# LiyaoTang/contrastBoundary

Hardware: AMD Instinct MI355X
Metric: points/sec through KNN+group+KPConv+CBL block, S3DIS N=40960 K=16 (higher is better)
Workload: dtype f32

## Files before the change

contrastboundary_amd/build.py:

```python
import concurrent.futures
import os
import shutil
import subprocess
import sys

PKG = os.path.dirname(os.path.abspath(__file__))
CSRC = os.path.join(PKG, "csrc")
LIBDIR = os.path.join(PKG, "lib")
OBJDIR = os.path.join(LIBDIR, "obj")
SO = os.path.join(LIBDIR, "libcbl_amd.so")
INCLUDE = os.path.join(os.path.dirname(PKG), "include")

HIPCC = shutil.which("hipcc") or "/opt/rocm/bin/hipcc"
FLAGS = ["--offload-arch=gfx950", "-O3", "-std=c++17", "-fPIC", "-ffp-contract=off", "-munsafe-fp-atomics",
         "-fvisibility=hidden", "-Wall", "-Wno-unused-function", "-I" + INCLUDE, "-I" + CSRC]


def sources():
    return sorted(os.path.join(CSRC, f) for f in os.listdir(CSRC) if f.endswith(".hip"))


def headers():
    hs = [os.path.join(CSRC, f) for f in os.listdir(CSRC) if f.endswith(".h")]
    hs += [os.path.join(INCLUDE, f) for f in os.listdir(INCLUDE) if f.endswith(".h")]
    return hs


EXTRA_FLAGS = {"local_aggregation.hip": ["-mllvm", "-amdgpu-mfma-vgpr-form"]}

def _compile(src, obj, verbose):
    tmp = obj + ".tmp.%d" % os.getpid()
    cmd = [HIPCC] + FLAGS + EXTRA_FLAGS.get(os.path.basename(src), []) + ["-c", src, "-o", tmp]
    if verbose:
        print(" ".join(cmd), flush=True)
    r = subprocess.run(cmd, capture_output=True, text=True)
    if r.returncode != 0:
        raise RuntimeError("hipcc failed for %s:\n%s\n%s" % (src, r.stdout, r.stderr))
    if verbose and r.stderr.strip():
        print(r.stderr)
    os.replace(tmp, obj)


def is_stale():
    if not os.path.exists(SO):
        return True
    t = os.path.getmtime(SO)
    return any(os.path.getmtime(p) > t for p in sources() + headers())


def build(force=False, verbose=False):
    import fcntl
    os.makedirs(OBJDIR, exist_ok=True)
    with open(os.path.join(LIBDIR, ".build.lock"), "w") as lock:
        fcntl.flock(lock, fcntl.LOCK_EX)
        try:
            if not force and not is_stale():
                return SO
            return _build_locked(force, verbose)
        finally:
            fcntl.flock(lock, fcntl.LOCK_UN)


def _build_locked(force, verbose):
    hdr_time = max([os.path.getmtime(h) for h in headers()] + [os.path.getmtime(__file__)])
    jobs, objs = [], []
    for src in sources():
        obj = os.path.join(OBJDIR, os.path.basename(src)[:-4] + ".o")
        objs.append(obj)
        if force or not os.path.exists(obj) or os.path.getmtime(obj) < max(os.path.getmtime(src), hdr_time):
            jobs.append((src, obj))
    if jobs:
        with concurrent.futures.ThreadPoolExecutor(max_workers=min(8, len(jobs))) as ex:
            for f in [ex.submit(_compile, s, o, verbose) for s, o in jobs]:
                f.result()
    if jobs or not os.path.exists(SO):
        tmp = SO + ".tmp.%d" % os.getpid()
        cmd = [HIPCC, "--offload-arch=gfx950", "-shared", "-fPIC", "-o", tmp] + objs
        if verbose:
            print(" ".join(cmd), flush=True)
        r = subprocess.run(cmd, capture_output=True, text=True)
        if r.returncode != 0:
            raise RuntimeError("link failed:\n%s\n%s" % (r.stdout, r.stderr))
        os.replace(tmp, SO)
    else:
        os.utime(SO)
    return SO


if __name__ == "__main__":
    print(build(force="--force" in sys.argv, verbose="--verbose" in sys.argv))
```

contrastboundary_amd/csrc/local_aggregation.hip:

```cpp
#include "cbl_common.h"

namespace {

using f32x4 = __attribute__((ext_vector_type(4))) float;

template <bool VEC>
__global__ __launch_bounds__(256) void kpconv_fwd_kernel(int n, int n0, int K, int C, int KP, const float* __restrict__ q,
                                                         const float* __restrict__ s, const int* __restrict__ idx, const float* __restrict__ f,
                                                         const float* __restrict__ kpts, const float* __restrict__ kw, float extent,
                                                         int influence, int closest, const int* __restrict__ order, float* __restrict__ out)
{
    const int lane = threadIdx.x & 63;
    const int kp_id = lane & 15;
    const int kq = lane >> 4;
    const unsigned wv = __builtin_amdgcn_readfirstlane(threadIdx.x >> 6), nwg = ((unsigned)n + 3u) >> 2;
    const bool kp_ok = kp_id < KP;
    const float kx = kp_ok ? kpts[3 * kp_id] : 0.f, ky = kp_ok ? kpts[3 * kp_id + 1] : 0.f, kz = kp_ok ? kpts[3 * kp_id + 2] : 0.f;

    const float inv_extent = 1.0f / extent;
    const unsigned vend = 8 * cbl_xcd_per(nwg), vstep = gridDim.x;
    auto point_at = [&](unsigned v) -> int {
        if (v >= vend) return -1;
        const unsigned t = (order ? cbl_xcd_slot(v, nwg) : v) * 4 + wv;
        return t < (unsigned)n ? (order ? order[t] : (int)t) : -1;
    };
    struct Geo { int id; float sx, sy, sz, qx, qy, qz; };
    auto fetch_ids = [&](int pt, Geo& g) {
        g.id = (lane < K) ? idx[(size_t)pt * K + lane] : n0;
        g.qx = q[3 * pt]; g.qy = q[3 * pt + 1]; g.qz = q[3 * pt + 2];
    };
    auto fetch_xyz = [&](Geo& g) {
        const bool real = g.id >= 0 && g.id < n0;
        const float3 sp = *reinterpret_cast<const float3*>(s + 3 * (size_t)(real ? g.id : 0));
        g.sx = real ? sp.x : 1e6f; g.sy = real ? sp.y : 1e6f; g.sz = real ? sp.z : 1e6f;
    };
    int p0 = point_at(blockIdx.x), p1 = point_at(blockIdx.x + vstep);
    Geo cur = {n0, 1e6f, 1e6f, 1e6f, 0.f, 0.f, 0.f};
    if (p0 >= 0) { fetch_ids(p0, cur); fetch_xyz(cur); }
    for (unsigned v = blockIdx.x; v < vend; v += vstep) {
        const int p2 = point_at(v + 2 * vstep);
        Geo nxt = {n0, 1e6f, 1e6f, 1e6f, 0.f, 0.f, 0.f};
        if (p1 >= 0) fetch_ids(p1, nxt);
        const int p = p0;
        const Geo g = cur;
        auto advance = [&]() { if (p1 >= 0) fetch_xyz(nxt); cur = nxt; p0 = p1; p1 = p2; };
        if (p < 0) { advance(); continue; }
        const float qx = g.qx, qy = g.qy, qz = g.qz;
        for (int c0 = 0; c0 < C; c0 += 64) {
            f32x4 acc[4];
#pragma unroll
            for (int t = 0; t < 4; t++) acc[t] = f32x4{0.f, 0.f, 0.f, 0.f};
            const int cb = c0 + 4 * kp_id;
            for (int k0 = 0; k0 < K; k0 += 64) {
                int my_id; float mrx, mry, mrz;
                if (k0 == 0) { my_id = g.id; mrx = g.sx - qx; mry = g.sy - qy; mrz = g.sz - qz; }
                else {
                    const int my_nb = k0 + lane;
                    my_id = (my_nb < K) ? idx[(size_t)p * K + my_nb] : n0;
                    const bool my_real = my_id >= 0 && my_id < n0;
                    mrx = (my_real ? s[3 * my_id] : 1e6f) - qx; mry = (my_real ? s[3 * my_id + 1] : 1e6f) - qy; mrz = (my_real ? s[3 * my_id + 2] : 1e6f) - qz;
                }
                const int kend = min(64, K - k0);
                for (int kc = 0; kc < kend; kc += 16) {
                    float bv[4][4]; float a[4];
#pragma unroll
                    for (int g = 0; g < 4; g++) {
                        const int src = kc + 4 * g + kq;
                        const int id = __shfl(my_id, src & 63);
                        const bool in = (kc + 4 * g + kq) < kend;
                        const bool real = in && id >= 0 && id < n0;
#pragma unroll
                        for (int t = 0; t < 4; t++) bv[g][t] = 0.f;
                        if (real) {
                            if (VEC) {
                                if (cb < C) { const float4 v = *reinterpret_cast<const float4*>(f + (size_t)id * C + cb); bv[g][0] = v.x; bv[g][1] = v.y; bv[g][2] = v.z; bv[g][3] = v.w; }
                            } else {
#pragma unroll
                                for (int t = 0; t < 4; t++) if (cb + t < C) bv[g][t] = f[(size_t)id * C + cb + t];
                            }
                        }
                        const float rx = __shfl(mrx, src & 63), ry = __shfl(mry, src & 63), rz = __shfl(mrz, src & 63);
                        const float dx = rx - kx, dy = ry - ky, dz = rz - kz;
                        const float sq = (dx * dx + dy * dy) + dz * dz;
                        float w = influence ? fmaxf(1.0f - __builtin_amdgcn_sqrtf(sq) * inv_extent, 0.0f) : 1.0f;
                        if (closest) {
                            float bs = kp_ok ? sq : INFINITY; int bi = kp_id;
#pragma unroll
                            for (int sft = 8; sft >= 1; sft >>= 1) {
                                const float os = __shfl_xor(bs, sft, 16); const int oi = __shfl_xor(bi, sft, 16);
                                if (os < bs || (os == bs && oi < bi)) { bs = os; bi = oi; }
                            }
                            if (bi != kp_id) w = 0.f;
                        }
                        a[g] = (kp_ok && in) ? w : 0.f;
                    }
#pragma unroll
                    for (int g = 0; g < 4; g++)
#pragma unroll
                        for (int t = 0; t < 4; t++) acc[t] = __builtin_amdgcn_mfma_f32_16x16x4f32(a[g], bv[g][t], acc[t], 0, 0, 0);
                }
            }
            float res[4];
#pragma unroll
            for (int t = 0; t < 4; t++) {
                float part = 0.f;
#pragma unroll
                for (int r = 0; r < 4; r++) {
                    const int row = kq * 4 + r;
                    const float kwv = (row < KP && cb + t < C) ? kw[(size_t)row * C + cb + t] : 0.f;
                    part += kwv * acc[t][r];
                }
                part += __shfl_xor(part, 16);
                part += __shfl_xor(part, 32);
                res[t] = part;
            }
            if (lane < 16) {
                if (VEC) { if (cb < C) *reinterpret_cast<float4*>(out + (size_t)p * C + cb) = make_float4(res[0], res[1], res[2], res[3]); }
                else {
#pragma unroll
                    for (int t = 0; t < 4; t++) if (cb + t < C) out[(size_t)p * C + cb + t] = res[t];
                }
            }
        }
        advance();
    }
}

__device__ __forceinline__ float rows_sum4(float x)
{
    const unsigned u = __float_as_uint(x);
    const auto a = __builtin_amdgcn_permlane16_swap(u, u, false, false);
    const float y = __uint_as_float(a[0]) + __uint_as_float(a[1]);
    const unsigned w = __float_as_uint(y);
    const auto b = __builtin_amdgcn_permlane32_swap(w, w, false, false);
    return __uint_as_float(b[0]) + __uint_as_float(b[1]);
}

template <bool CLOSEST, bool LINEAR, bool ONE>
__global__ __launch_bounds__(256) void kpconv_fwd_c64_kernel(int n, int n0, int K, int C, int KP, const float* __restrict__ q,
                                                             const float* __restrict__ s, const int* __restrict__ idx, const float* __restrict__ f,
                                                             const float* __restrict__ kpts, const float* __restrict__ kw, float extent,
                                                             const int* __restrict__ order, float* __restrict__ out)
{
    __shared__ float4 kw_s[16 * 16];
    {
        const int row = threadIdx.x >> 4, col = threadIdx.x & 15;
        kw_s[threadIdx.x] = (row < KP && 4 * col < C) ? *reinterpret_cast<const float4*>(kw + (size_t)row * C + 4 * col) : make_float4(0.f, 0.f, 0.f, 0.f);
    }
    __syncthreads();
    const int lane = threadIdx.x & 63;
    const int kp_id = lane & 15, kq = lane >> 4;
    const unsigned wv = __builtin_amdgcn_readfirstlane(threadIdx.x >> 6), nwg = ((unsigned)n + 3u) >> 2;
    const bool kp_ok = kp_id < KP;
    const float kx = kp_ok ? kpts[3 * kp_id] : 0.f, ky = kp_ok ? kpts[3 * kp_id + 1] : 0.f, kz = kp_ok ? kpts[3 * kp_id + 2] : 0.f;
    const float inv_extent = 1.0f / extent;
    const float m2kx = -2.f * kx, m2ky = -2.f * ky, m2kz = -2.f * kz, k2 = (kx * kx + ky * ky) + kz * kz;
    const int cb = 4 * kp_id;
    const bool ch_ok = cb < C;
    const char* fbytes = reinterpret_cast<const char*>(f);
    const unsigned row_bytes = 4u * (unsigned)C, col_bytes = 4u * (unsigned)(ch_ok ? cb : 0);
    const unsigned vend = 8 * cbl_xcd_per(nwg), vstep = gridDim.x;
    auto point_at = [&](unsigned v) -> int {
        if (v >= vend) return -1;
        const unsigned t = (order ? cbl_xcd_slot(v, nwg) : v) * 4 + wv;
        return t < (unsigned)n ? (order ? order[t] : (int)t) : -1;
    };
    struct Xyz { float x, y, z, qx, qy, qz; };
    struct Rows { float4 v[4]; bool real[4]; };
    auto load_ids = [&](int pt) -> int { return (pt >= 0 && lane < K) ? idx[(size_t)pt * K + lane] : n0; };
    auto load_xyz = [&](int pt, int id) -> Xyz {
        Xyz g;
        const bool real = id >= 0 && id < n0;
        const float3 sp = *reinterpret_cast<const float3*>(s + 3 * (size_t)(real ? id : 0));
        g.x = real ? sp.x : 1e6f; g.y = real ? sp.y : 1e6f; g.z = real ? sp.z : 1e6f;
        const float3 qp = *reinterpret_cast<const float3*>(q + 3 * (size_t)(pt >= 0 ? pt : 0));
        g.qx = qp.x; g.qy = qp.y; g.qz = qp.z;
        return g;
    };
    auto load_rows = [&](int ids, int kc) -> Rows {
        Rows r;
#pragma unroll
        for (int gi = 0; gi < 4; gi++) {
            const int id = __shfl(ids, (kc + 4 * gi + kq) & 63);
            r.real[gi] = id >= 0 && id < n0;
            r.v[gi] = *reinterpret_cast<const float4*>(fbytes + ((unsigned)(r.real[gi] ? id : 0) * row_bytes + col_bytes));
        }
        return r;
    };
    const f32x4 zero = {0.f, 0.f, 0.f, 0.f};
    auto chunk = [&](const Rows& rows, int kc, float mrx, float mry, float mrz, float mr2, f32x4 (&acc)[4], bool first) {
        float a[4];
#pragma unroll
        for (int gi = 0; gi < 4; gi++) {
            const int src = (kc + 4 * gi + kq) & 63;
            const float rx = __shfl(mrx, src), ry = __shfl(mry, src), rz = __shfl(mrz, src);
            float sq;
            if (CLOSEST) {
                const float dx = rx - kx, dy = ry - ky, dz = rz - kz;
                sq = (dx * dx + dy * dy) + dz * dz;
            } else {
                const float r2 = __shfl(mr2, src);
                sq = fmaxf(__builtin_fmaf(m2kx, rx, __builtin_fmaf(m2ky, ry, __builtin_fmaf(m2kz, rz, r2 + k2))), 0.f);
            }
            float w = LINEAR ? fmaxf(1.0f - __builtin_amdgcn_sqrtf(sq) * inv_extent, 0.0f) : 1.0f;
            if (CLOSEST) {
                float bs = kp_ok ? sq : INFINITY; int bi = kp_id;
#pragma unroll
                for (int sft = 8; sft >= 1; sft >>= 1) {
                    const float os = __shfl_xor(bs, sft, 16); const int oi = __shfl_xor(bi, sft, 16);
                    if (os < bs || (os == bs && oi < bi)) { bs = os; bi = oi; }
                }
                if (bi != kp_id) w = 0.f;
            }
            a[gi] = (kp_ok && rows.real[gi]) ? w : 0.f;
        }
#pragma unroll
        for (int gi = 0; gi < 4; gi++) {
            const bool z = first && gi == 0;
            const bool rl = rows.real[gi];
            acc[0] = __builtin_amdgcn_mfma_f32_16x16x4f32(a[gi], rl ? rows.v[gi].x : 0.f, z ? zero : acc[0], 0, 0, 0);
            acc[1] = __builtin_amdgcn_mfma_f32_16x16x4f32(a[gi], rl ? rows.v[gi].y : 0.f, z ? zero : acc[1], 0, 0, 0);
            acc[2] = __builtin_amdgcn_mfma_f32_16x16x4f32(a[gi], rl ? rows.v[gi].z : 0.f, z ? zero : acc[2], 0, 0, 0);
            acc[3] = __builtin_amdgcn_mfma_f32_16x16x4f32(a[gi], rl ? rows.v[gi].w : 0.f, z ? zero : acc[3], 0, 0, 0);
        }
    };
    int p0 = point_at(blockIdx.x), p1 = point_at(blockIdx.x + vstep), p2 = point_at(blockIdx.x + 2 * vstep);
    int id0 = load_ids(p0), id1 = load_ids(p1);
    Xyz g0 = load_xyz(p0, id0);
    Rows r0 = load_rows(id0, 0);
    for (unsigned v = blockIdx.x; v < vend; v += vstep) {
        const int p3 = point_at(v + 3 * vstep);
        const int p = p0;
        const int id2 = load_ids(p2); const Xyz g1 = load_xyz(p1, id1); const Rows r1 = load_rows(id1, 0);
        __builtin_amdgcn_sched_barrier(0);
        if (p >= 0) {
            const float mrx = g0.x - g0.qx, mry = g0.y - g0.qy, mrz = g0.z - g0.qz;
            const float mr2 = (mrx * mrx + mry * mry) + mrz * mrz;
            f32x4 acc[4];
#pragma unroll
            for (int t = 0; t < 4; t++) acc[t] = zero;
            chunk(r0, 0, mrx, mry, mrz, mr2, acc, true);
            if (!ONE) {
                for (int k0 = 0; k0 < K; k0 += 64) {
                    int ids = id0; float cx = mrx, cy = mry, cz = mrz, c2 = mr2;
                    if (k0 > 0) {
                        ids = (k0 + lane < K) ? idx[(size_t)p * K + k0 + lane] : n0;
                        const bool real = ids >= 0 && ids < n0;
                        const float3 sp = *reinterpret_cast<const float3*>(s + 3 * (size_t)(real ? ids : 0));
                        cx = (real ? sp.x : 1e6f) - g0.qx; cy = (real ? sp.y : 1e6f) - g0.qy; cz = (real ? sp.z : 1e6f) - g0.qz;
                        c2 = (cx * cx + cy * cy) + cz * cz;
                    }
                    for (int kc = (k0 == 0 ? 16 : 0); kc < min(64, K - k0); kc += 16) {
                        const Rows rr = load_rows(ids, kc);
                        chunk(rr, kc, cx, cy, cz, c2, acc, false);
                    }
                }
            }
            float res[4];
#pragma unroll
            for (int t = 0; t < 4; t++) res[t] = 0.f;
#pragma unroll
            for (int r = 0; r < 4; r++) {
                const float4 k4 = kw_s[(kq * 4 + r) * 16 + kp_id];
                res[0] = __builtin_fmaf(k4.x, acc[0][r], res[0]); res[1] = __builtin_fmaf(k4.y, acc[1][r], res[1]);
                res[2] = __builtin_fmaf(k4.z, acc[2][r], res[2]); res[3] = __builtin_fmaf(k4.w, acc[3][r], res[3]);
            }
#pragma unroll
            for (int t = 0; t < 4; t++) res[t] = rows_sum4(res[t]);
            if (lane < 16 && ch_ok) *reinterpret_cast<float4*>(out + (size_t)p * C + cb) = make_float4(res[0], res[1], res[2], res[3]);
        }
        p0 = p1; p1 = p2; p2 = p3; id0 = id1; id1 = id2; g0 = g1; r0 = r1;
    }
}

constexpr int KPB_MAXKP = 16, KPB_MAXK = 64;
__global__ __launch_bounds__(256) void kpconv_bwd_kernel(int n, int n0, int K, int C, int KP, const float* __restrict__ q,
                                                         const float* __restrict__ s, const int* __restrict__ idx, const float* __restrict__ f,
                                                         const float* __restrict__ kpts, const float* __restrict__ kw, float extent,
                                                         int influence, int closest, const float* __restrict__ go,
                                                         float* __restrict__ gf, float* __restrict__ gkw)
{
    __shared__ float w_s[4][KPB_MAXKP * KPB_MAXK];
    __shared__ int id_s[4][KPB_MAXK];
    const int lane = threadIdx.x & 63, wv = threadIdx.x >> 6;
    const int wave0 = __builtin_amdgcn_readfirstlane((blockIdx.x * 256 + threadIdx.x) >> 6), nwaves = (gridDim.x * 256) >> 6;
    float* W = w_s[wv]; int* ID = id_s[wv];
    for (int c0 = 0; c0 < C; c0 += 64) {
        const int c = c0 + lane;
        const bool cok = c < C;
        float kwr[KPB_MAXKP], gacc[KPB_MAXKP];
#pragma unroll
        for (int kp = 0; kp < KPB_MAXKP; kp++) { kwr[kp] = (cok && kp < KP) ? kw[(size_t)kp * C + c] : 0.f; gacc[kp] = 0.f; }
        for (int p = wave0; p < n; p += nwaves) {
            const float qx = q[3 * p], qy = q[3 * p + 1], qz = q[3 * p + 2];
            for (int k = lane; k < K; k += 64) ID[k] = idx[(size_t)p * K + k];
            for (int e = lane; e < KP * K; e += 64) {
                const int kp = e / K, k = e - kp * K;
                const int id = idx[(size_t)p * K + k];
                const bool real = id >= 0 && id < n0;
                const float rx = (real ? s[3 * id] : 1e6f) - qx, ry = (real ? s[3 * id + 1] : 1e6f) - qy, rz = (real ? s[3 * id + 2] : 1e6f) - qz;
                const float dx = rx - kpts[3 * kp], dy = ry - kpts[3 * kp + 1], dz = rz - kpts[3 * kp + 2];
                const float sq = (dx * dx + dy * dy) + dz * dz;
                float w = influence ? fmaxf(1.0f - sqrtf(sq) / extent, 0.0f) : 1.0f;
                if (closest) {
                    for (int o = 0; o < KP; o++) {
                        const float ex = rx - kpts[3 * o], ey = ry - kpts[3 * o + 1], ez = rz - kpts[3 * o + 2];
                        const float osq = (ex * ex + ey * ey) + ez * ez;
                        if (osq < sq || (osq == sq && o < kp)) { w = 0.f; break; }
                    }
                }
                W[kp * K + k] = w;
            }
            __builtin_amdgcn_s_waitcnt(0xc07f);
            __builtin_amdgcn_wave_barrier();
            const float g = cok ? go[(size_t)p * C + c] : 0.f;
            float wf[KPB_MAXKP];
#pragma unroll
            for (int kp = 0; kp < KPB_MAXKP; kp++) wf[kp] = 0.f;
            for (int k = 0; k < K; k++) {
                const int id = ID[k];
                const bool real = id >= 0 && id < n0;
                const float fk = (real && cok) ? f[(size_t)id * C + c] : 0.f;
                float coef = 0.f;
#pragma unroll
                for (int kp = 0; kp < KPB_MAXKP; kp++) {
                    const float w = (kp < KP) ? W[kp * K + k] : 0.f;
                    wf[kp] += w * fk;
                    coef += w * kwr[kp];
                }
                if (real && cok && gf) unsafeAtomicAdd(gf + (size_t)id * C + c, g * coef);
            }
#pragma unroll
            for (int kp = 0; kp < KPB_MAXKP; kp++) gacc[kp] += g * wf[kp];
        }
        if (gkw && cok)
            for (int kp = 0; kp < KP; kp++) unsafeAtomicAdd(gkw + (size_t)kp * C + c, gacc[kp]);
    }
}

__global__ __launch_bounds__(256) void index_max_kernel(long long total, int vec, const int* __restrict__ idx, int* __restrict__ out)
{
    __shared__ int red[4];
    int m = -2147483647 - 1;
    const long long gid = (long long)blockIdx.x * 256 + threadIdx.x, stride = (long long)gridDim.x * 256;
    const long long t4 = vec ? (total >> 2) : 0;
    const int4* __restrict__ v = reinterpret_cast<const int4*>(idx);
    for (long long e = gid; e < t4; e += stride) { const int4 x = v[e]; m = max(m, max(max(x.x, x.y), max(x.z, x.w))); }
    for (long long e = 4 * t4 + gid; e < total; e += stride) m = max(m, idx[e]);
    for (int s = 32; s >= 1; s >>= 1) m = max(m, __shfl_xor(m, s));
    if ((threadIdx.x & 63) == 0) red[threadIdx.x >> 6] = m;
    __syncthreads();
    if (threadIdx.x == 0) atomicMax(out, max(max(red[0], red[1]), max(red[2], red[3])));
}

template <bool BWD>
__global__ __launch_bounds__(256) void adaptive_weight_kernel(int n, int n0, int K, int C, const float* __restrict__ q, const float* __restrict__ s,
                                                              const int* __restrict__ idx, const float* __restrict__ f, float radius,
                                                              const float* __restrict__ fcw, const float* __restrict__ fcb,
                                                              const int* __restrict__ padding_num, int reduction_mean,
                                                              float* __restrict__ out,
                                                              const float* __restrict__ go, float* __restrict__ gf,
                                                              float* __restrict__ gfcw, float* __restrict__ gfcb)
{
    const int lane = threadIdx.x & 63;
    const int wave0 = __builtin_amdgcn_readfirstlane((blockIdx.x * 256 + threadIdx.x) >> 6), nwaves = (gridDim.x * 256) >> 6;
    const int pad = reduction_mean ? *padding_num : 0;
    for (int c0 = 0; c0 < C; c0 += 64) {
        const int c = c0 + lane;
        const bool cok = c < C;
        const float w0 = cok ? fcw[c] : 0.f, w1 = cok ? fcw[C + c] : 0.f, w2 = cok ? fcw[2 * C + c] : 0.f, bb = cok ? fcb[c] : 0.f;
        float a0 = 0.f, a1 = 0.f, a2 = 0.f, ab = 0.f;
        for (int p = wave0; p < n; p += nwaves) {
            const float qx = q[3 * p], qy = q[3 * p + 1], qz = q[3 * p + 2];
            float nn = 1.f;
            if (reduction_mean) {
                int cnt = 0;
                for (int k = lane; k < K; k += 64) cnt += idx[(size_t)p * K + k] < pad ? 1 : 0;
                for (int sft = 32; sft >= 1; sft >>= 1) cnt += __shfl_xor(cnt, sft);
                nn = (float)cnt + 1e-5f;
            }
            const float g = (BWD && cok) ? go[(size_t)p * C + c] / nn : 0.f;
            float acc = 0.f;
            for (int k = 0; k < K; k++) {
                const int id = idx[(size_t)p * K + k];
                const bool real = id >= 0 && id < n0;
                const float rx = ((real ? s[3 * id] : 0.f) - qx) / radius, ry = ((real ? s[3 * id + 1] : 0.f) - qy) / radius,
                            rz = ((real ? s[3 * id + 2] : 0.f) - qz) / radius;
                const float w = ((rx * w0 + ry * w1) + rz * w2) + bb;
                const float fk = (real && cok) ? f[(size_t)id * C + c] : 0.f;
                if (!BWD) acc += w * fk;
                else {
                    if (real && cok && gf) unsafeAtomicAdd(gf + (size_t)id * C + c, g * w);
                    const float gw = g * fk;
                    a0 += gw * rx; a1 += gw * ry; a2 += gw * rz; ab += gw;
                }
            }
            if (!BWD && cok) out[(size_t)p * C + c] = acc / nn;
        }
        if (BWD && cok) {
            if (gfcw) { unsafeAtomicAdd(gfcw + c, a0); unsafeAtomicAdd(gfcw + C + c, a1); unsafeAtomicAdd(gfcw + 2 * C + c, a2); }
            if (gfcb) unsafeAtomicAdd(gfcb + c, ab);
        }
    }
}

template <int U>
__global__ __launch_bounds__(256) void adaptive_weight_fwd_v4(unsigned n, int n0, int K, int C4, int c4_0, int L, const float* __restrict__ q, const float* __restrict__ s,
                                                              const int* __restrict__ idx, const float4* __restrict__ f, float inv_radius,
                                                              const float4* __restrict__ fcw, const float4* __restrict__ fcb,
                                                              const int* __restrict__ padding_num, int reduction_mean, const int* __restrict__ order,
                                                              float4* __restrict__ out)
{
    const int pad = reduction_mean ? *padding_num : 0;
    const int tpb = 256 / L;
    const int ts = threadIdx.x / L, cl = threadIdx.x - ts * L;
    if (ts >= tpb) return;
    const int cq = c4_0 + cl;
    const float4 w0 = fcw[cq], w1 = fcw[C4 + cq], w2 = fcw[2 * C4 + cq], bb = fcb[cq];
    const unsigned ntrips = (n + tpb - 1) / tpb;
    const unsigned vend = 8 * cbl_xcd_per(ntrips);
    for (unsigned v = blockIdx.x; v < vend; v += gridDim.x) {
        const unsigned tr = cbl_xcd_slot(v, ntrips) * tpb + ts;
        if (tr >= n) continue;
        const int p = order ? order[tr] : (int)tr;
        const float qx = q[3 * (size_t)p], qy = q[3 * (size_t)p + 1], qz = q[3 * (size_t)p + 2];
        const int* __restrict__ row = idx + (size_t)p * K;
        float4 acc = make_float4(0.f, 0.f, 0.f, 0.f);
        int cnt = 0;
        int idn[U];
#pragma unroll
        for (int u = 0; u < U; u++) { const int v_ = row[min(u, K - 1)]; idn[u] = (u < K) ? v_ : n0; }
        for (int k0 = 0; k0 < K; k0 += U) {
            int id[U]; float rx[U], ry[U], rz[U]; float4 fk[U];
#pragma unroll
            for (int u = 0; u < U; u++) {
                id[u] = idn[u];
                cnt += (k0 + u < K && id[u] < pad) ? 1 : 0;
            }
#pragma unroll
            for (int u = 0; u < U; u++) { const int v_ = row[min(k0 + U + u, K - 1)]; idn[u] = (k0 + U + u < K) ? v_ : n0; }
#pragma unroll
            for (int u = 0; u < U; u++) {
                const bool real = id[u] >= 0 && id[u] < n0;
                const int ic = real ? id[u] : 0;
                fk[u] = f[(size_t)ic * C4 + cq];
                rx[u] = s[3 * (size_t)ic]; ry[u] = s[3 * (size_t)ic + 1]; rz[u] = s[3 * (size_t)ic + 2];
                if (!real) { fk[u] = make_float4(0.f, 0.f, 0.f, 0.f); rx[u] = ry[u] = rz[u] = 0.f; }
            }
#pragma unroll
            for (int u = 0; u < U; u++) {
                if (k0 + u < K) {
                    const float x = (rx[u] - qx) * inv_radius, y = (ry[u] - qy) * inv_radius, z = (rz[u] - qz) * inv_radius;
                    acc.x += (((x * w0.x + y * w1.x) + z * w2.x) + bb.x) * fk[u].x;
                    acc.y += (((x * w0.y + y * w1.y) + z * w2.y) + bb.y) * fk[u].y;
                    acc.z += (((x * w0.z + y * w1.z) + z * w2.z) + bb.z) * fk[u].z;
                    acc.w += (((x * w0.w + y * w1.w) + z * w2.w) + bb.w) * fk[u].w;
                }
            }
        }
        const float nn = reduction_mean ? (float)cnt + 1e-5f : 1.f;
        out[(size_t)p * C4 + cq] = make_float4(acc.x / nn, acc.y / nn, acc.z / nn, acc.w / nn);
    }
}

template <int CPL, int U>
__global__ __launch_bounds__(256) void adaptive_weight_fwd_v5(unsigned n, int n0, int K, int C4, int c4_0, int L, const float* __restrict__ q, const float* __restrict__ s,
                                                              const int* __restrict__ idx, const float4* __restrict__ f, float inv_radius,
                                                              const float4* __restrict__ fcw, const float4* __restrict__ fcb,
                                                              const int* __restrict__ padding_num, int reduction_mean, const int* __restrict__ order,
                                                              float4* __restrict__ out)
{
    const int pad = reduction_mean ? *padding_num : 0;
    const int tpb = 256 / L;
    const int ts = threadIdx.x / L, cl = threadIdx.x - ts * L;
    if (ts >= tpb) return;
    const int cq = c4_0 + cl * CPL;
    const unsigned ntrips = (n + tpb - 1) / tpb;
    const unsigned vend = 8 * cbl_xcd_per(ntrips);
    for (unsigned v = blockIdx.x; v < vend; v += gridDim.x) {
        const unsigned tr = cbl_xcd_slot(v, ntrips) * tpb + ts;
        if (tr >= n) continue;
        const int p = order ? order[tr] : (int)tr;
        const float qx = q[3 * (size_t)p], qy = q[3 * (size_t)p + 1], qz = q[3 * (size_t)p + 2];
        const int* __restrict__ row = idx + (size_t)p * K;
        float4 S0[CPL], S1[CPL], S2[CPL], S3[CPL];
#pragma unroll
        for (int j = 0; j < CPL; j++) S0[j] = S1[j] = S2[j] = S3[j] = make_float4(0.f, 0.f, 0.f, 0.f);
        int cnt = 0;
        int idn[U];
#pragma unroll
        for (int u = 0; u < U; u++) { const int v_ = row[min(u, K - 1)]; idn[u] = (u < K) ? v_ : n0; }
        for (int k0 = 0; k0 < K; k0 += U) {
            int id[U]; float rx[U], ry[U], rz[U]; float4 fk[U][CPL];
#pragma unroll
            for (int u = 0; u < U; u++) {
                id[u] = idn[u];
                cnt += (k0 + u < K && id[u] < pad) ? 1 : 0;
            }
#pragma unroll
            for (int u = 0; u < U; u++) { const int v_ = row[min(k0 + U + u, K - 1)]; idn[u] = (k0 + U + u < K) ? v_ : n0; }
#pragma unroll
            for (int u = 0; u < U; u++) {
                const bool real = id[u] >= 0 && id[u] < n0;
                const int ic = real ? id[u] : 0;
                const float4* __restrict__ fr = f + (size_t)ic * C4 + cq;
#pragma unroll
                for (int j = 0; j < CPL; j++) fk[u][j] = fr[j];
                rx[u] = s[3 * (size_t)ic]; ry[u] = s[3 * (size_t)ic + 1]; rz[u] = s[3 * (size_t)ic + 2];
            }
#pragma unroll
            for (int u = 0; u < U; u++) {
                const bool real = id[u] >= 0 && id[u] < n0;
                const float one = real ? 1.f : 0.f;
                const float x = real ? (rx[u] - qx) * inv_radius : 0.f, y = real ? (ry[u] - qy) * inv_radius : 0.f, z = real ? (rz[u] - qz) * inv_radius : 0.f;
#pragma unroll
                for (int j = 0; j < CPL; j++) {
                    const float4 fv = fk[u][j];
                    S0[j] = make_float4(fmaf(x, fv.x, S0[j].x), fmaf(x, fv.y, S0[j].y), fmaf(x, fv.z, S0[j].z), fmaf(x, fv.w, S0[j].w));
                    S1[j] = make_float4(fmaf(y, fv.x, S1[j].x), fmaf(y, fv.y, S1[j].y), fmaf(y, fv.z, S1[j].z), fmaf(y, fv.w, S1[j].w));
                    S2[j] = make_float4(fmaf(z, fv.x, S2[j].x), fmaf(z, fv.y, S2[j].y), fmaf(z, fv.z, S2[j].z), fmaf(z, fv.w, S2[j].w));
                    S3[j] = make_float4(fmaf(one, fv.x, S3[j].x), fmaf(one, fv.y, S3[j].y), fmaf(one, fv.z, S3[j].z), fmaf(one, fv.w, S3[j].w));
                }
            }
        }
        const float inv_nn = reduction_mean ? 1.0f / ((float)cnt + 1e-5f) : 1.f;
#pragma unroll
        for (int j = 0; j < CPL; j++) {
            const float4 w0 = fcw[cq + j], w1 = fcw[C4 + cq + j], w2 = fcw[2 * C4 + cq + j], bb = fcb[cq + j];
            float4 o;
            o.x = fmaf(bb.x, S3[j].x, fmaf(w2.x, S2[j].x, fmaf(w1.x, S1[j].x, w0.x * S0[j].x))) * inv_nn;
            o.y = fmaf(bb.y, S3[j].y, fmaf(w2.y, S2[j].y, fmaf(w1.y, S1[j].y, w0.y * S0[j].y))) * inv_nn;
            o.z = fmaf(bb.z, S3[j].z, fmaf(w2.z, S2[j].z, fmaf(w1.z, S1[j].z, w0.z * S0[j].z))) * inv_nn;
            o.w = fmaf(bb.w, S3[j].w, fmaf(w2.w, S2[j].w, fmaf(w1.w, S1[j].w, w0.w * S0[j].w))) * inv_nn;
            out[(size_t)p * C4 + cq + j] = o;
        }
    }
}

__global__ __launch_bounds__(256) void aw_inv_count_kernel(int n, int K, const int* __restrict__ idx, const int* __restrict__ padding_num,
                                                           int reduction_mean, float* __restrict__ inv_nn)
{
    const int pad = reduction_mean ? *padding_num : 0;
    for (int p = blockIdx.x * 256 + threadIdx.x; p < n; p += gridDim.x * 256) {
        int cnt = 0;
        if (reduction_mean)
            for (int k = 0; k < K; k++) cnt += idx[(size_t)p * K + k] < pad ? 1 : 0;
        inv_nn[p] = reduction_mean ? 1.0f / ((float)cnt + 1e-5f) : 1.0f;
    }
}

template <bool GF, bool GP, int UB, int CPL>
__global__ __launch_bounds__(256) void aw_bwd_csr_kernel(unsigned n0, int C4, int c4_0, int L, CblFastDiv dvK, const float* __restrict__ q, const float* __restrict__ s,
                                                        const float4* __restrict__ f, float inv_radius, const float4* __restrict__ fcw, const float4* __restrict__ fcb,
                                                        const float* __restrict__ inv_nn, const float4* __restrict__ go,
                                                        const int* __restrict__ order, const int* __restrict__ inv_start, const int* __restrict__ inv_src,
                                                        float4* __restrict__ gf, float* __restrict__ partial)
{
    __shared__ float4 red[4][256];
    const int tpb = 256 / L;
    const int ts = threadIdx.x / L, cl = threadIdx.x - ts * L;
    const bool on = ts < tpb;
    const int cq = c4_0 + cl * CPL;
    float4 A[4][CPL];
#pragma unroll
    for (int a = 0; a < 4; a++)
#pragma unroll
        for (int c = 0; c < CPL; c++) A[a][c] = make_float4(0.f, 0.f, 0.f, 0.f);
    const unsigned ntrips = (n0 + tpb - 1) / tpb;
    const unsigned vend = 8 * cbl_xcd_per(ntrips);
    for (unsigned v = blockIdx.x; v < vend; v += gridDim.x) {
        const unsigned tr = cbl_xcd_slot(v, ntrips) * tpb + ts;
        if (!on || tr >= n0) continue;
        const int j = order ? order[tr] : (int)tr;
        const int e0 = inv_start[tr], e1 = inv_start[tr + 1];
        const float sx = s[3 * (size_t)j], sy = s[3 * (size_t)j + 1], sz = s[3 * (size_t)j + 2];
        float4 S0[CPL], S1[CPL], S2[CPL], S3[CPL];
// ... 450 lines not shown
```

contrastboundary_amd/csrc/query_group_pipe.h:

```cpp
#pragma once
#include <gather_wave.h>

constexpr int QGP_WAVES = 4;

template <int C4T, int PR>
__global__ __launch_bounds__(256) void query_group_lds_pipe(unsigned npieces, const float* __restrict__ xyz, const float* __restrict__ new_xyz,
                                                            const float4* __restrict__ feat, const int* __restrict__ idx, const int* __restrict__ order,
                                                            float* __restrict__ out)
{
    constexpr int oc = 4 * C4T + 3, NF4 = PR * C4T, NL = (NF4 + 63) / 64, NCH = PR * oc / 4, NS = (NCH + 63) / 64, NC = (3 * PR + 63) / 64;
    static_assert((PR * oc) % 4 == 0 && NF4 % 64 == 0, "pieces are whole 16-byte chunks, feature parts whole wave loads");
    __shared__ __attribute__((aligned(16))) float qg_lds[QGP_WAVES * PR * oc];
    const int lane = threadIdx.x & 63, wv = gw_uniform((int)(threadIdx.x >> 6));
    float* piece = qg_lds + wv * PR * oc;
    const unsigned nwg = (npieces + 3) >> 2, vend = 8 * cbl_xcd_per(nwg), vstep = gridDim.x;
    auto piece_of = [&](unsigned v) -> int {
        const unsigned t = (v < vend ? cbl_xcd_slot(v, nwg) : 0u) * 4 + wv;
        const bool ok = v < vend && t < npieces;
        const int pt = order[ok ? t : 0u];
        return gw_uniform(ok ? pt : -1);
    };
    auto ids_of = [&](int pc) -> int { return idx[(size_t)(pc < 0 ? 0 : pc) * PR + (lane < PR ? lane : 0)]; };
    float4 v[NL]; float cs[NC], cq[NC];
    auto load_piece = [&](int ids, int pc) {
        const int pq = pc < 0 ? 0 : pc;
#pragma unroll
        for (int j = 0; j < NL; j++) {
            const int f = lane + 64 * j, row = f / C4T, part = f % C4T;
            v[j] = feat[(size_t)gw_shfl(ids, row) * C4T + part];
        }
#pragma unroll
        for (int h = 0; h < NC; h++) {
            const int e = 64 * h + lane, ec = e < 3 * PR ? e : 0, row = ec / 3, a = ec - 3 * row;
            cs[h] = xyz[(size_t)gw_shfl(ids, row) * 3 + a];
            cq[h] = new_xyz[(size_t)pq * 3 + a];
        }
    };
    auto park = [&]() {
#pragma unroll
        for (int j = 0; j < NL; j++) {
            const int f = lane + 64 * j, row = f / C4T, part = f % C4T;
            float* d = piece + row * oc + 3 + 4 * part;
            d[0] = v[j].x; d[1] = v[j].y; d[2] = v[j].z; d[3] = v[j].w;
        }
#pragma unroll
        for (int h = 0; h < NC; h++) {
            const int e = 64 * h + lane, row = e / 3, a = e - 3 * row;
            if (e < 3 * PR) piece[row * oc + a] = cs[h] - cq[h];
        }
    };
    int p0 = piece_of(blockIdx.x), p1 = piece_of(blockIdx.x + vstep), p2 = piece_of(blockIdx.x + 2 * vstep);
    int id1 = ids_of(p1);
    load_piece(ids_of(p0), p0);
    park();
    int pc = p0;
    p0 = p1; { const int idn = id1; p1 = p2; id1 = ids_of(p1); p2 = piece_of(blockIdx.x + 3 * vstep); load_piece(idn, p0); }
    for (unsigned vv = blockIdx.x; vv < vend; vv += vstep) {
        gw_wave_sync();
        {
            float* o = out + (size_t)(pc < 0 ? 0 : pc) * PR * oc;
#pragma unroll
            for (int u = 0; u < NS; u++) {
                const int ch = lane + 64 * u;
                if (ch < NCH) gw_store16_streaming(o + 4 * ch, piece + 4 * ch);
            }
        }
        gw_wave_sync();
        park();
        pc = p0;
        p0 = p1; const int idn = id1; p1 = p2;
        id1 = ids_of(p1);
        p2 = piece_of(vv + 4 * vstep);
        load_piece(idn, p0);
    }
}
```

contrastboundary_amd/hotpath.py:

```python
import os
import sys

import torch

from . import heads, local_aggregation, pointops

KP = 15
CBL_NSAMPLE = 36
CBL_DIM = 32


class Scene:

    def __init__(self, xyz, feat, labels, offset):
        self.xyz, self.feat, self.labels, self.offset = xyz, feat, labels, offset
        self.n, self.c = feat.shape

    @staticmethod
    def synthetic_numpy(n, c, seed=0, b=1):
        import numpy as np
        from . import synthetic as S
        xyz, labels = S.s_room(n, seed, scale=1.0 if n <= 100000 else float(np.sqrt(n / 40000.0)))
        rng = np.random.default_rng(seed + 1000)
        feat = rng.normal(size=(n, c)).astype(np.float32)
        off = S.offsets(n, b, seed)
        kpts = (rng.normal(size=(KP, 3)) * 0.06).astype(np.float32); kpts[0] = 0
        kw = (rng.normal(size=(KP, c)) / np.sqrt(KP)).astype(np.float32)
        latent = rng.normal(size=(n, CBL_DIM)).astype(np.float32)
        return dict(xyz=xyz, feat=feat, labels=labels, offset=off, kernel_points=kpts, kernel_weights=kw, latent=latent)

    @staticmethod
    def upstream_numpy(n, c, k, seed=0):
        import numpy as np
        rng = np.random.default_rng(seed + 2000)
        return dict(grad_grouped=rng.normal(size=(n, k, 3 + c)).astype(np.float32), grad_kpconv=rng.normal(size=(n, c)).astype(np.float32))

    @staticmethod
    def synthetic(n, c, seed=0, b=1, device="cuda"):
        a = Scene.synthetic_numpy(n, c, seed, b)
        t = lambda v: torch.from_numpy(v).to(device)
        sc = Scene(t(a["xyz"]), t(a["feat"]), t(a["labels"]), t(a["offset"]))
        sc.kernel_points, sc.kernel_weights, sc.latent = t(a["kernel_points"]), t(a["kernel_weights"]), t(a["latent"])
        sc.seed = seed
        return sc

    def upstream(self, k):
        cache = self.__dict__.setdefault("_upstream", {})
        if k not in cache:
            a = Scene.upstream_numpy(self.n, self.c, k, getattr(self, "seed", 0))
            cache[k] = {name: torch.from_numpy(v).to(self.xyz.device) for name, v in a.items()}
        return cache[k]


SIDE_STAGES = ("cbl_knnquery_k%d" % CBL_NSAMPLE,)


def stages(scene, k=16, backward=False, pair_tables=False):
    n, c = scene.n, scene.c
    st = []
    leaf = (lambda t: t.detach().requires_grad_(True)) if backward else (lambda t: t)
    if backward:
        scene.upstream(k)

    def knn(s):
        s["idx"], s["dist2"] = pointops.knnquery_raw(k, scene.xyz, scene.xyz, scene.offset, scene.offset)
    st.append(("knnquery_k%d" % k, knn, 12 * n + 12 * n + 8 * n * k, 8.0 * n * n))

    def group(s):
        s["feat_leaf"], s["kw_leaf"] = leaf(scene.feat), leaf(scene.kernel_weights)
        s["grouped"] = pointops.queryandgroup(k, scene.xyz, scene.xyz, s["feat_leaf"], s["idx"], scene.offset, scene.offset, use_xyz=True)
    st.append(("queryandgroup", group, 4 * n * k + 12 * n + 12 * n + 4 * n * c + 4 * n * k * (3 + c), 3.0 * n * k))

    extent = 0.12

    def kpconv(s):
        s["kpconv"] = local_aggregation.kpconv(scene.xyz, scene.xyz, s["idx"], s["feat_leaf"], scene.kernel_points, s["kw_leaf"], extent)
    st.append(("kpconv_fwd", kpconv, 12 * n + 12 * n + 4 * n * c + 4 * n * k + 4 * n * c, 2.0 * n * k * KP * c + 2.0 * n * KP * c))

    d = CBL_DIM

    def cbl_knn(s):
        s["cbl_idx"], _ = pointops.knnquery_raw(CBL_NSAMPLE, scene.xyz, scene.xyz, scene.offset, scene.offset, algo="set")
    st.append(("cbl_knnquery_k%d" % CBL_NSAMPLE, cbl_knn, 24 * n + 8 * n * CBL_NSAMPLE, 8.0 * n * n))

    def cbl_transpose(s):
        s["cbl_transposed"] = pointops.neighbor_transpose(s["cbl_idx"], n, companion=s.get("idx") if (pair_tables and backward) else None)
    st.append(("cbl_neighbor_transpose", cbl_transpose, 8 * n * CBL_NSAMPLE + 4 * (n + 1), 0.0))

    def cbl_fwd(s):
        s["cbl_latent"] = scene.latent.detach().requires_grad_(True)
        s["cbl_loss"] = heads.point_contrast(s["cbl_latent"], scene.labels, s["cbl_idx"], 1.0, 0.1)
    st.append(("cbl_mining_loss_fwd", cbl_fwd, 4 * n * CBL_NSAMPLE + 4 * n * d + 4 * n + 8 * n + 4 * n * CBL_NSAMPLE + 4 * n * d,
               1.0 * n * (CBL_NSAMPLE - 1) * (8 * d + 50)))

    def cbl_bwd(s):
        s["cbl_grad"], = torch.autograd.grad(s["cbl_loss"], s["cbl_latent"])
    st.append(("cbl_mining_loss_bwd", cbl_bwd, 4 * (n + 1) + 8 * n * CBL_NSAMPLE + 12 * n * d, 3.0 * n * (CBL_NSAMPLE - 1) * d))
    if not backward:
        return st

    def transpose(s):
        s["transposed"] = pointops.neighbor_transpose(s["idx"], n)
    st.append(("neighbor_transpose_k%d" % k, transpose, 8 * n * k + 4 * (n + 1), 0.0))

    def group_bwd(s):
        s["grad_feat_group"], = torch.autograd.grad(s["grouped"], s["feat_leaf"], scene.upstream(k)["grad_grouped"])
    st.append(("queryandgroup_bwd", group_bwd, 4 * n * k + 4 * n * k * c + 4 * n * c, 1.0 * n * k * c))

    def kpconv_bwd(s):
        s["grad_feat_kpconv"], s["grad_kernel_weights"] = torch.autograd.grad(s["kpconv"], (s["feat_leaf"], s["kw_leaf"]), scene.upstream(k)["grad_kpconv"])
    st.append(("kpconv_bwd", kpconv_bwd, 12 * n + 12 * n + 4 * n * c + 4 * n * k + 4 * n * c + 4 * n * c + 4 * KP * c,
               2.0 * (2.0 * n * k * KP * c + 2.0 * n * KP * c)))
    return st


def pt_layer(scene, seed=0):
    from . import blocks
    cache = scene.__dict__.setdefault("_pt_layer", {})
    if seed not in cache:
        torch.manual_seed(1234 + seed)
        cache[seed] = blocks.PointTransformerLayer(scene.c, scene.c, 8, 16).to(scene.xyz.device).train()
    return cache[seed]


def stages_pt(scene, k=16, backward=False, pair_tables=False):
    n, c = scene.n, scene.c
    layer = pt_layer(scene)
    layer.nsample = k
    params = [p for p in layer.parameters()]
    st = []
    if backward:
        scene.upstream(k)

    def knn(s):
        s["idx"], s["dist2"] = pointops.knnquery_raw(k, scene.xyz, scene.xyz, scene.offset, scene.offset)
    st.append(("knnquery_k%d" % k, knn, 12 * n + 12 * n + 8 * n * k, 8.0 * n * n))

    def layer_fwd(s):
        s["feat_leaf"] = scene.feat.detach().requires_grad_(True) if backward else scene.feat
        s["pt_out"] = layer([scene.xyz, s["feat_leaf"], scene.offset], idx=s["idx"])
    st.append(("pt_layer_fwd", layer_fwd, 12 * n + 12 * n * c + 4 * n * k + 4 * n * c,
               2.0 * n * k * (9 + 3 * c + c * c / 8.0 + c * c / 64.0) + 6.0 * n * c * c))

    d = CBL_DIM

    def cbl_knn(s):
        s["cbl_idx"], _ = pointops.knnquery_raw(CBL_NSAMPLE, scene.xyz, scene.xyz, scene.offset, scene.offset, algo="set")
    st.append(("cbl_knnquery_k%d" % CBL_NSAMPLE, cbl_knn, 24 * n + 8 * n * CBL_NSAMPLE, 8.0 * n * n))

    def cbl_transpose(s):
        s["cbl_transposed"] = pointops.neighbor_transpose(s["cbl_idx"], n, companion=s.get("idx") if (pair_tables and backward) else None)
    st.append(("cbl_neighbor_transpose", cbl_transpose, 8 * n * CBL_NSAMPLE + 4 * (n + 1), 0.0))

    def cbl_fwd(s):
        s["cbl_latent"] = scene.latent.detach().requires_grad_(True)
        s["cbl_loss"] = heads.point_contrast(s["cbl_latent"], scene.labels, s["cbl_idx"], 1.0, 0.1)
    st.append(("cbl_mining_loss_fwd", cbl_fwd, 4 * n * CBL_NSAMPLE + 4 * n * d + 4 * n + 8 * n + 4 * n * CBL_NSAMPLE + 4 * n * d,
               1.0 * n * (CBL_NSAMPLE - 1) * (8 * d + 50)))

    def cbl_bwd(s):
        s["cbl_grad"], = torch.autograd.grad(s["cbl_loss"], s["cbl_latent"])
    st.append(("cbl_mining_loss_bwd", cbl_bwd, 4 * (n + 1) + 8 * n * CBL_NSAMPLE + 12 * n * d, 3.0 * n * (CBL_NSAMPLE - 1) * d))
    if not backward:
        return st

    def transpose(s):
        s["transposed"] = pointops.neighbor_transpose(s["idx"], n)
    st.append(("neighbor_transpose_k%d" % k, transpose, 8 * n * k + 4 * (n + 1), 0.0))

    def layer_bwd(s):
        grads = torch.autograd.grad(s["pt_out"], [s["feat_leaf"]] + params, scene.upstream(k)["grad_kpconv"])
        s["grad_feat_pt"], s["grad_params_pt"] = grads[0], grads[1:]
    st.append(("pt_layer_bwd", layer_bwd, 12 * n + 12 * n * c + 4 * n * k + 4 * n * c + 4 * n * c + 4 * sum(p.numel() for p in params),
               2.0 * (2.0 * n * k * (9 + 3 * c + c * c / 8.0 + c * c / 64.0) + 6.0 * n * c * c)))
    return st


def search_hints(scene):
    return ((scene.xyz, CBL_NSAMPLE, "set"),)


def run_once(scene, k=16, state=None, backward=False):
    state = {} if state is None else state
    for _, fn, _, _ in stages(scene, k, backward):
        fn(state)
    return state


class Schedule:

    def __init__(self, stage_list, overlap=True, hints=(), aux_tables=True, pair_tables=False):
        self.stage_list = stage_list
        self.pair_tables = pair_tables
        self.aux_tables = aux_tables
        self.hints = tuple(hints)
        self.overlap = overlap
        self.side = torch.cuda.Stream() if overlap else None
        self.aux = []
        self.joined = torch.cuda.Event() if overlap else None

    def run(self, state, events=None, side_after=None):
        if self.hints:
            with pointops.neighbor_cache() as nc:
                nc.record_events = self.overlap
                for xyz, nsample, algo in self.hints:
                    nc.hint(xyz, nsample, algo)
                return self._run_branches(state, events) if self.overlap else self._run(state, events, None, ())
        return self._run(state, events, side_after, SIDE_STAGES if self.overlap else ())

    def _join_table(self, name, state):
        key = "cbl_idx" if name.startswith("cbl_") else "idx"
        if name in ("cbl_mining_loss_bwd", "queryandgroup_bwd", "pt_layer_bwd") and key in state:
            pointops.neighbor_transpose(state[key], state[key].shape[0], build=False)

    def _launch(self, i, state, events):
        if self.overlap:
            self._join_table(self.stage_list[i][0], state)
        if events is not None:
            events[i][0].record()
        self.stage_list[i][1](state)
        if events is not None:
            events[i][1].record()

    def _run_branches(self, state, events):
        main = torch.cuda.current_stream()
        names = [st[0] for st in self.stage_list]
        tr_idx = [i for i, nm in enumerate(names) if "neighbor_transpose" in nm and not nm.startswith("cbl_")] if self.aux_tables else []
        side_idx = [i for i, nm in enumerate(names) if nm.startswith("cbl_")]
        main_idx = [i for i in range(len(names)) if i not in side_idx and i not in tr_idx]
        while len(self.aux) < len(tr_idx):
            self.aux.append(torch.cuda.Stream())
        self.side.wait_stream(main)
        self._launch(main_idx[0], state, events)
        before = {key: id(v) for key, v in state.items()}
        aux_of = {i: self.aux[n] for n, i in enumerate(tr_idx)}
        for i in tr_idx:
            aux_of[i].wait_stream(main)
            with torch.cuda.stream(aux_of[i]):
                self._launch(i, state, events)
        with torch.cuda.stream(self.side):
            for i in side_idx:
                self._launch(i, state, events)
            self.joined.record(self.side)
        for i in main_idx[1:]:
            self._launch(i, state, events)
        main.wait_event(self.joined)
        for i in tr_idx:
            main.wait_stream(aux_of[i])
        for key, v in state.items():
            if before.get(key) != id(v):
                for t in (v if isinstance(v, (tuple, list)) else (v,)):
                    if torch.is_tensor(t):
                        t.record_stream(main)
        return state

    def _run(self, state, events, side_after, side_names):
        main = torch.cuda.current_stream()
        names = [st[0] for st in self.stage_list]
        side_idx = [i for i, nm in enumerate(names) if nm in side_names]
        fork_at = names.index(side_after) if (side_after is not None and side_idx) else -1
        produced = []

        def fork():
            self.side.wait_stream(main)
            before = {key: id(v) for key, v in state.items()}
            with torch.cuda.stream(self.side):
                for i in side_idx:
                    self._launch(i, state, events)
                self.joined.record(self.side)
            produced.extend(v for key, v in state.items() if torch.is_tensor(v) and before.get(key) != id(v))
        if side_idx and fork_at < 0:
            fork()
        waited = not side_idx
        for i in range(len(names)):
            if i in side_idx:
                continue
            if not waited and i > side_idx[-1]:
                main.wait_event(self.joined)
                for v in produced:
                    v.record_stream(main)
                waited = True
            self._launch(i, state, events)
            if i == fork_at:
                fork()
        if not waited:
            main.wait_event(self.joined)
        return state


def concurrent_streams(count, candidates=12, spin_cycles=2_000_000, beside=None):
    def timed(streams):
        torch.cuda.synchronize()
        t0, t1 = torch.cuda.Event(enable_timing=True), torch.cuda.Event(enable_timing=True)
        cur = torch.cuda.current_stream()
        t0.record(cur)
        for s in streams:
            s.wait_event(t0)
        for s in streams:
            with torch.cuda.stream(s):
                torch.cuda._sleep(spin_cycles)
        for s in set(streams):
            cur.wait_stream(s)
        t1.record(cur)
        torch.cuda.synchronize()
        return t0.elapsed_time(t1)

    debug = os.environ.get("CBL_STREAM_PROBE_DEBUG")

    def together(a, b):
        for _ in range(2):
            s0 = timed([a, a]); pair = timed([a, b]); s1 = timed([a, a])
            if debug:
                print("probe: serial %.3f pair %.3f serial %.3f ms -> %s" % (s0, pair, s1, pair < 0.75 * min(s0, s1)), file=sys.stderr)
            if not pair < 0.75 * min(s0, s1):
                return False
        return True
    pool = [torch.cuda.Stream() for _ in range(candidates)]
    if not hasattr(torch.cuda, "_sleep"):
        return pool[:count]
    last = None
    for _ in range(60):
        for _ in range(8):
            torch.cuda._sleep(spin_cycles)
        t = timed([pool[0]])
        if last is not None and abs(t - last) < 0.02 * last:
            break
        last = t
    fixed = [] if beside is None else (list(beside) if isinstance(beside, (list, tuple)) else [beside])
    chosen = []
    for s in pool:
        if len(chosen) == count:
            break
        if all(together(c, s) for c in fixed + chosen):
            chosen.append(s)
    if len(chosen) < count:
        chosen += [p for p in pool if p not in chosen][:count - len(chosen)]
    return chosen


class Pipeline:

    SLOTS = 3
    LAYOUT = "split_t36_first"

    @staticmethod
    def plan(names, layout):
        ix = lambda pred: [i for i, nm in enumerate(names) if pred(nm)]
        search = ix(lambda nm: "knnquery" in nm)
        t16 = ix(lambda nm: "neighbor_transpose" in nm and not nm.startswith("cbl_"))
        t36 = ix(lambda nm: "neighbor_transpose" in nm and nm.startswith("cbl_"))
        cbl = [i for i in ix(lambda nm: nm.startswith("cbl_")) if i not in search and i not in t36]
        block = [i for i in range(len(names)) if i not in search + t16 + t36 + cbl]
        bwd = lambda i: names[i].endswith("_bwd")
        fwd_b, bwd_b = [i for i in block if not bwd(i)], [i for i in block if bwd(i)]
        fwd_c, bwd_c = [i for i in cbl if not bwd(i)], [i for i in cbl if bwd(i)]
        if layout == "tables":
            streams = ("search", "tables", "rest", "side")
            segs = [("search", "search", search, (), "found"),
                    ("t16", "tables", t16, ("found",), "t16"),
                    ("fwd", "rest", fwd_b, ("found",), None),
                    ("cblfwd", "side", fwd_c, ("found",), None),
                    ("t36", "tables", t36, ("found",), "t36"),
                    ("bwd", "rest", bwd_b, ("t16",) if t16 else (), None),
                    ("cblbwd", "side", bwd_c, ("t36",) if t36 else (), None)]
        elif layout == "split_t36_first":
            streams = ("search", "fwd", "bwd", "side")
            segs = [("search", "search", search, (), "found"),
                    ("fwd", "fwd", fwd_b, ("found",), "fdone"),
                    ("cbl", "side", t36 + fwd_c + bwd_c, ("found",), None),
                    ("bwd", "bwd", t16 + bwd_b, ("fdone",), None)]
        elif layout == "alt_bwd":
            streams = ("search", "fwd", "bwd0", "bwd1")
            segs = [("search", "search", search, (), "found"),
                    ("fwd", "fwd", fwd_b + t16, ("found",), "fdone"),
                    ("cbl", "search", t36 + fwd_c + bwd_c, (), None),
                    ("bwd", "bwd*", bwd_b, ("fdone",), None)]
        elif layout == "pair_split":
            streams = ("search", "fwd", "bwd", "side")
            segs = [("search", "search", search, (), "found"),
                    ("fwd", "fwd", fwd_b, ("found",), "fdone"),
                    ("tabs", "side", t36, ("found",), "tabs"),
                    ("cbl", "side", fwd_c + bwd_c, (), None),
                    ("bwd", "bwd", t16 + bwd_b, ("fdone", "tabs") if t36 else ("fdone",), None)]
        elif layout == "pair_alt_bwd":
            streams = ("search", "fwd", "bwd0", "bwd1")
            segs = [("search", "search", search, (), "found"),
                    ("fwd", "fwd", fwd_b, ("found",), "fdone"),
                    ("tabs", "search", t36, (), "tabs"),
                    ("cbl", "search", fwd_c + bwd_c, (), None),
                    ("bwd", "bwd*", t16 + bwd_b, ("fdone", "tabs") if t36 else ("fdone",), None)]
        else:
            raise ValueError("unknown pipeline layout %r" % layout)
        return streams, [sg for sg in segs if sg[2]]

    def __init__(self, sched, layout=None, slots=None):
        import os
        assert sched.hints, "the pipeline is built on the one-search-per-geometry schedule"
        self.sched = sched
        self.layout = layout or os.environ.get("CBL_PIPELINE_LAYOUT", self.LAYOUT)
        self.SLOTS = int(slots or os.environ.get("CBL_PIPELINE_SLOTS", self.SLOTS))
        if self.layout.startswith("pair_") != bool(getattr(sched, "pair_tables", False)):
            raise ValueError("pipeline layout %r does not fit a step whose stages were made with pair_tables=%s" % (self.layout, bool(getattr(sched, "pair_tables", False))))
        self.STREAMS, self.segments = self.plan([st[0] for st in sched.stage_list], self.layout)
        self.streams = dict(zip(self.STREAMS, concurrent_streams(len(self.STREAMS))))
        self.states = [{} for _ in range(self.SLOTS)]
        self.graphs = [dict() for _ in range(self.SLOTS)]
        recorded = sorted({sg[4] for sg in self.segments if sg[4]})
        self.events = [{nm: torch.cuda.Event() for nm in recorded} for _ in range(self.SLOTS)]
        self.done = [{c: torch.cuda.Event() for c in self.STREAMS[1:]} for _ in range(self.SLOTS)]
        self.count = 0

    def describe(self):
# ... 62 lines not shown
```

contrastboundary_amd/local_aggregation.py:

```python
import collections
import ctypes

import torch
from torch.autograd import Function

from . import _lib

_i = ctypes.c_int
_f = ctypes.c_float


def _chk(t, dtype, name):
    if not (isinstance(t, torch.Tensor) and t.is_cuda and t.dtype == dtype and t.is_contiguous()):
        raise TypeError(f"{name}: expected a contiguous CUDA tensor of {dtype}")
    return t


class _KPConv(Function):
    @staticmethod
    def forward(ctx, query_points, support_points, neighbors_indices, features, kernel_points, kernel_weights, extent, influence, closest):
        n, K = neighbors_indices.shape
        n0, C = features.shape
        KP = kernel_points.shape[0]
        out = torch.empty((n, C), dtype=torch.float32, device=features.device)
        from . import pointops
        order = pointops.spatial_order(query_points)
        _lib.check(_lib.lib().cbl_kpconv_forward_ordered(_i(n), _i(n0), _i(K), _i(C), _i(KP), _lib.ptr(query_points), _lib.ptr(support_points),
                                                         _lib.ptr(neighbors_indices), _lib.ptr(features), _lib.ptr(kernel_points), _lib.ptr(kernel_weights),
                                                         _f(extent), _i(influence), _i(closest), _lib.ptr(order), _lib.ptr(out),
                                                         _lib.stream_of(features)), "cbl_kpconv_forward")
        ctx.save_for_backward(query_points, support_points, neighbors_indices, features, kernel_points, kernel_weights)
        ctx.cfg = (extent, influence, closest)
        return out

    @staticmethod
    def backward(ctx, grad_out):
        q, s, idx, f, kp, kw = ctx.saved_tensors
        extent, influence, closest = ctx.cfg
        n, K = idx.shape
        n0, C = f.shape
        grad_out = grad_out.contiguous()
        L = _lib.lib()
        from . import pointops
        tr = None
        if C % 4 == 0:
            tr = pointops.neighbor_transpose(idx, n0, build=pointops._build_table(n * K))
        if tr is not None:
            order, inv_start, inv_src = tr
            gf = torch.empty_like(f) if ctx.needs_input_grad[3] else None
            gkw = torch.empty_like(kw) if ctx.needs_input_grad[5] else None
            need = L.cbl_kpconv_backward_csr_workspace_bytes(_i(n0), _i(C), _i(kp.shape[0])) if gkw is not None else 0
            ws = torch.empty(max(need, 1), dtype=torch.uint8, device=f.device)
            rc = L.cbl_kpconv_backward_csr(_i(n), _i(n0), _i(K), _i(C), _i(kp.shape[0]), _lib.ptr(q), _lib.ptr(s), _lib.ptr(f), _lib.ptr(kp), _lib.ptr(kw),
                                           _f(extent), _i(influence), _i(closest), _lib.ptr(grad_out), _lib.ptr(order), _lib.ptr(inv_start), _lib.ptr(inv_src),
                                           _lib.ptr(gf), _lib.ptr(gkw), _lib.ptr(ws), ctypes.c_size_t(ws.numel()), _lib.stream_of(f))
            if rc != _lib.ERR_UNSUPPORTED:
                _lib.check(rc, "cbl_kpconv_backward_csr")
                return None, None, None, gf, None, gkw, None, None, None
        gf = torch.zeros_like(f) if ctx.needs_input_grad[3] else None
        gkw = torch.zeros_like(kw) if ctx.needs_input_grad[5] else None
        _lib.check(L.cbl_kpconv_backward(_i(n), _i(n0), _i(K), _i(C), _i(kp.shape[0]), _lib.ptr(q), _lib.ptr(s), _lib.ptr(idx), _lib.ptr(f),
                                         _lib.ptr(kp), _lib.ptr(kw), _f(extent), _i(influence), _i(closest), _lib.ptr(grad_out),
                                         _lib.ptr(gf), _lib.ptr(gkw), _lib.stream_of(f)), "cbl_kpconv_backward")
        return None, None, None, gf, None, gkw, None, None, None


def kpconv(query_points, support_points, neighbors_indices, features, kernel_points, kernel_weights, extent,
           KP_influence="linear", convolution_mode="sum"):
    _chk(query_points, torch.float32, "query_points"); _chk(support_points, torch.float32, "support_points")
    _chk(neighbors_indices, torch.int32, "neighbors_indices"); _chk(features, torch.float32, "features")
    _chk(kernel_points, torch.float32, "kernel_points"); _chk(kernel_weights, torch.float32, "kernel_weights")
    if KP_influence not in ("linear", "constant"):
        raise NotImplementedError("KP_influence 'gaussian': radius_gaussian is not defined in the reference")
    if convolution_mode not in ("sum", "closest"):
        raise ValueError("Unknown convolution mode. Should be 'closest' or 'sum'")
    return _KPConv.apply(query_points, support_points, neighbors_indices, features, kernel_points, kernel_weights, float(extent),
                         1 if KP_influence == "linear" else 0, 1 if convolution_mode == "closest" else 0)


class _AdaptiveWeight(Function):
    @staticmethod
    def forward(ctx, query_points, support_points, neighbors_indices, features, fc_weight, fc_bias, radius, reduction_mean):
        n, K = neighbors_indices.shape
        n0, C = features.shape
        L = _lib.lib()
        pad = torch.empty(1, dtype=torch.int32, device=features.device)
        if reduction_mean:
            _lib.check(L.cbl_index_max(ctypes.c_longlong(n * K), _lib.ptr(neighbors_indices), _lib.ptr(pad), _lib.stream_of(features)), "cbl_index_max")
        out = torch.empty((n, C), dtype=torch.float32, device=features.device)
        from . import pointops
        order = pointops.spatial_order(query_points)
        _lib.check(L.cbl_adaptive_weight_forward_ordered(_i(n), _i(n0), _i(K), _i(C), _lib.ptr(query_points), _lib.ptr(support_points), _lib.ptr(neighbors_indices),
                                                         _lib.ptr(features), _f(radius), _lib.ptr(fc_weight), _lib.ptr(fc_bias), _lib.ptr(pad), _i(reduction_mean),
                                                         _lib.ptr(order), _lib.ptr(out), _lib.stream_of(features)), "cbl_adaptive_weight_forward")
        ctx.save_for_backward(query_points, support_points, neighbors_indices, features, fc_weight, fc_bias, pad)
        ctx.cfg = (radius, reduction_mean)
        return out

    @staticmethod
    def backward(ctx, grad_out):
        q, s, idx, f, w, b, pad = ctx.saved_tensors
        radius, reduction_mean = ctx.cfg
        n, K = idx.shape
        n0, C = f.shape
        grad_out = grad_out.contiguous()
        L = _lib.lib()
        need_f, need_w, need_b = ctx.needs_input_grad[3], ctx.needs_input_grad[4], ctx.needs_input_grad[5]
        from . import pointops
        tr = None
        if C % 4 == 0:
            tr = pointops.neighbor_transpose(idx, n0, build=pointops._build_table(n * K))
        if tr is not None:
            order, inv_start, inv_src = tr
            gf = torch.empty_like(f) if need_f else None
            gw = torch.empty_like(w) if need_w else None
            gb = torch.empty_like(b) if need_b else None
            ws = torch.empty(L.cbl_adaptive_weight_backward_csr_workspace_bytes(_i(n), _i(n0), _i(C)), dtype=torch.uint8, device=f.device)
            rc = L.cbl_adaptive_weight_backward_csr(_i(n), _i(n0), _i(K), _i(C), _lib.ptr(q), _lib.ptr(s), _lib.ptr(idx), _lib.ptr(f), _f(radius), _lib.ptr(w),
                                                    _lib.ptr(b), _lib.ptr(pad), _i(reduction_mean), _lib.ptr(grad_out), _lib.ptr(order), _lib.ptr(inv_start),
                                                    _lib.ptr(inv_src), _lib.ptr(gf), _lib.ptr(gw), _lib.ptr(gb), _lib.ptr(ws), ctypes.c_size_t(ws.numel()),
                                                    _lib.stream_of(f))
            if rc != _lib.ERR_UNSUPPORTED:
                _lib.check(rc, "cbl_adaptive_weight_backward_csr")
                return None, None, None, gf, gw, gb, None, None
        gf = torch.zeros_like(f) if need_f else None
        gw = torch.zeros_like(w) if need_w else None
        gb = torch.zeros_like(b) if need_b else None
        _lib.check(L.cbl_adaptive_weight_backward(_i(n), _i(n0), _i(K), _i(C), _lib.ptr(q), _lib.ptr(s), _lib.ptr(idx), _lib.ptr(f), _f(radius),
                                                  _lib.ptr(w), _lib.ptr(b), _lib.ptr(pad), _i(reduction_mean), _lib.ptr(grad_out),
                                                  _lib.ptr(gf), _lib.ptr(gw), _lib.ptr(gb), _lib.stream_of(f)), "cbl_adaptive_weight_backward")
        return None, None, None, gf, gw, gb, None, None


ADAPTIVE_WEIGHT_INPUTS = ("dp", "df", "dp_df", "fj", "dp_fj", "fi_df", "dp_fi_df")
_AW_SOFTMAX = {None: 0, False: 0, "dense": 1, "sparse": 1, "mask": 1, "unmask": 2}
_AW_REDUCTIONS = {"sum": 0, "mean": 1, "avg": 1, "max": 2}
_NO_TABLE = "{}: no transposed neighbour table for more than 2^20 support points, and there is no scatter form"


def _aw_d_in(local_input_feature, in_fdim):
    blocks = local_input_feature.split("_")
    return 3 * ("dp" in blocks) + in_fdim * sum(b in blocks for b in ("fi", "df", "fj"))


def _aw_options(local_input_feature, shared_channels, weight_softmax, reduction, in_fdim):
    if local_input_feature not in ADAPTIVE_WEIGHT_INPUTS:
        raise NotImplementedError("local_input_feature {} not supported in AdaptiveWeight (one of {})".format(local_input_feature, ", ".join(ADAPTIVE_WEIGHT_INPUTS)))
    if weight_softmax not in _AW_SOFTMAX:
        raise NotImplementedError("weight_softmax {!r} not supported in AdaptiveWeight (False, 'dense', 'sparse', 'mask' or 'unmask')".format(weight_softmax))
    if reduction not in _AW_REDUCTIONS:
        raise NotImplementedError("Reduction {} not supported in AdaptiveWeight".format(reduction))
    S = min(int(shared_channels), in_fdim)
    if S < 1 or in_fdim % S != 0:
        raise NotImplementedError("shared_channels {}: {} features do not divide into groups of it (the reference's reshape fails as well)".format(shared_channels, in_fdim))
    if S not in (1, 2, 4) and S % 4 != 0:
        raise NotImplementedError("shared_channels {}: 1, 2, 4 or a multiple of 4".format(shared_channels))
    return S


class _AdaptiveWeightGeneral(Function):

    @staticmethod
    def forward(ctx, query_points, support_points, neighbors_indices, features, center_term, neighbor_term, w_pos, bias, radius, softmax, red):
        n, K = neighbors_indices.shape
        n0, C = features.shape
        M = bias.shape[0]
        L = _lib.lib()
        dev = features.device
        st = _lib.stream_of(features)
        pad = torch.empty(1, dtype=torch.int32, device=dev)
        if red == 1:
            _lib.check(L.cbl_index_max(ctypes.c_longlong(n * K), _lib.ptr(neighbors_indices), _lib.ptr(pad), st), "cbl_index_max")
        out = torch.empty((n, C), dtype=torch.float32, device=dev)
        _lib.check(L.cbl_adaptive_weight_general_forward(_i(n), _i(n0), _i(K), _i(C), _i(M), _lib.ptr(query_points), _lib.ptr(support_points),
                                                         _lib.ptr(neighbors_indices), _lib.ptr(features), _lib.ptr(center_term), _lib.ptr(neighbor_term),
                                                         _lib.ptr(w_pos), _lib.ptr(bias), _f(radius), _i(softmax), _i(red), _lib.ptr(pad), _lib.ptr(out),
                                                         None, ctypes.c_size_t(0), st), "cbl_adaptive_weight_general_forward")
        ctx.save_for_backward(query_points, support_points, neighbors_indices, features, center_term, neighbor_term, w_pos, bias, pad, out)
        ctx.cfg = (radius, softmax, red)
        return out

    @staticmethod
    def backward(ctx, grad_out):
        q, s, idx, f, cen, nbr, wp, bias, pad, out = ctx.saved_tensors
        radius, softmax, red = ctx.cfg
        n, K = idx.shape
        n0, C = f.shape
        M = bias.shape[0]
        grad_out = grad_out.contiguous()
        L = _lib.lib()
        dev = f.device
        st = _lib.stream_of(f)
        from . import pointops
        need = ctx.needs_input_grad
        new = lambda *shape: torch.empty(shape, dtype=torch.float32, device=dev)
        gf = new(n0, C) if need[3] else None
        gc = new(n, M) if cen is not None and need[4] else None
        gn = new(n0, M) if nbr is not None and need[5] else None
        gwp = new(3, M) if wp is not None and need[6] else None
        gb = new(M) if need[7] else None
        order = inv_start = inv_src = None
        if gf is not None or gn is not None:
            tr = pointops.neighbor_transpose(idx, n0, build=True)
            if tr is None:
                raise NotImplementedError(_NO_TABLE.format("adaptive_weight"))
            order, inv_start, inv_src = tr
        ws = torch.empty(max(L.cbl_adaptive_weight_general_workspace_bytes(_i(n), _i(n0), _i(K), _i(C), _i(M)), 1), dtype=torch.uint8, device=dev)
        _lib.check(L.cbl_adaptive_weight_general_backward_csr(_i(n), _i(n0), _i(K), _i(C), _i(M), _lib.ptr(q), _lib.ptr(s), _lib.ptr(idx), _lib.ptr(f),
                                                              _lib.ptr(cen), _lib.ptr(nbr), _lib.ptr(wp), _lib.ptr(bias), _f(radius), _i(softmax), _i(red),
                                                              _lib.ptr(pad), _lib.ptr(out), _lib.ptr(grad_out), _lib.ptr(order), _lib.ptr(inv_start),
                                                              _lib.ptr(inv_src), _lib.ptr(gf), _lib.ptr(gc), _lib.ptr(gn), _lib.ptr(gwp), _lib.ptr(gb),
                                                              _lib.ptr(ws), ctypes.c_size_t(ws.numel()), st), "cbl_adaptive_weight_general_backward_csr")
        gcen = None
        if gc is not None:
            tr0 = pointops.neighbor_transpose(idx[:, :1].contiguous(), n0, build=True)
            if tr0 is None:
                raise NotImplementedError(_NO_TABLE.format("adaptive_weight"))
            gcen = new(n0, M)
            _lib.check(L.cbl_grouping_backward_csr_rows(_i(n0), _i(M), _i(M), _i(0), _lib.ptr(gc), _lib.ptr(tr0[0]), _lib.ptr(tr0[1]), _lib.ptr(tr0[2]),
                                                        _lib.ptr(gcen), st), "cbl_grouping_backward_csr_rows")
        return None, None, None, gf, gcen, gn, gwp, gb, None, None, None


class _AdaptiveWeightMLP(Function):

    @staticmethod
    def forward(ctx, query_points, support_points, neighbors_indices, features, center_term, neighbor_term, w_pos, bias, hidden_w, hidden_b, radius, softmax,
                red, act):
        n, K = neighbors_indices.shape
        n0, C = features.shape
        M, layers = bias.shape[0], hidden_w.shape[0]
        L = _lib.lib()
        dev = features.device
        st = _lib.stream_of(features)
        pad = torch.empty(1, dtype=torch.int32, device=dev)
        if red == 1:
            _lib.check(L.cbl_index_max(ctypes.c_longlong(n * K), _lib.ptr(neighbors_indices), _lib.ptr(pad), st), "cbl_index_max")
        out = torch.empty((n, C), dtype=torch.float32, device=dev)
        _lib.check(L.cbl_adaptive_weight_mlp_forward(_i(n), _i(n0), _i(K), _i(C), _i(M), _lib.ptr(query_points), _lib.ptr(support_points),
                                                     _lib.ptr(neighbors_indices), _lib.ptr(features), _lib.ptr(center_term), _lib.ptr(neighbor_term),
                                                     _lib.ptr(w_pos), _lib.ptr(bias), _i(layers), _lib.ptr(hidden_w), _lib.ptr(hidden_b), _i(act), _f(radius),
                                                     _i(softmax), _i(red), _lib.ptr(pad), _lib.ptr(out), None, ctypes.c_size_t(0), st),
                   "cbl_adaptive_weight_mlp_forward")
        ctx.save_for_backward(query_points, support_points, neighbors_indices, features, center_term, neighbor_term, w_pos, bias, hidden_w, hidden_b, pad, out)
        ctx.cfg = (radius, softmax, red, act)
        return out

    @staticmethod
    def backward(ctx, grad_out):
        q, s, idx, f, cen, nbr, wp, bias, hw, hb, pad, out = ctx.saved_tensors
        radius, softmax, red, act = ctx.cfg
        n, K = idx.shape
        n0, C = f.shape
        M, layers = bias.shape[0], hw.shape[0]
        grad_out = grad_out.contiguous()
        L = _lib.lib()
        dev = f.device
        st = _lib.stream_of(f)
        from . import pointops
        need = ctx.needs_input_grad
        new = lambda *shape: torch.empty(shape, dtype=torch.float32, device=dev)
        gf = new(n0, C) if need[3] else None
        gc = new(n, M) if cen is not None and need[4] else None
        gn = new(n0, M) if nbr is not None and need[5] else None
        gwp = new(3, M) if wp is not None and need[6] else None
        gb = new(M) if need[7] else None
        ghw = new(layers, M, M) if need[8] else None
        ghb = new(layers, M) if need[9] else None
        order = inv_start = inv_src = None
        if gf is not None or gn is not None:
            tr = pointops.neighbor_transpose(idx, n0, build=True)
            if tr is None:
                raise NotImplementedError(_NO_TABLE.format("adaptive_weight"))
            order, inv_start, inv_src = tr
        ws = torch.empty(max(L.cbl_adaptive_weight_mlp_workspace_bytes(_i(n), _i(n0), _i(K), _i(C), _i(M), _i(layers)), 1), dtype=torch.uint8, device=dev)
        _lib.check(L.cbl_adaptive_weight_mlp_backward_csr(_i(n), _i(n0), _i(K), _i(C), _i(M), _lib.ptr(q), _lib.ptr(s), _lib.ptr(idx), _lib.ptr(f),
                                                          _lib.ptr(cen), _lib.ptr(nbr), _lib.ptr(wp), _lib.ptr(bias), _i(layers), _lib.ptr(hw), _lib.ptr(hb),
                                                          _i(act), _f(radius), _i(softmax), _i(red), _lib.ptr(pad), _lib.ptr(out), _lib.ptr(grad_out),
                                                          _lib.ptr(order), _lib.ptr(inv_start), _lib.ptr(inv_src), _lib.ptr(gf), _lib.ptr(gc), _lib.ptr(gn),
                                                          _lib.ptr(gwp), _lib.ptr(gb), _lib.ptr(ghw), _lib.ptr(ghb), _lib.ptr(ws),
                                                          ctypes.c_size_t(ws.numel()), st), "cbl_adaptive_weight_mlp_backward_csr")
        gcen = None
        if gc is not None:
            tr0 = pointops.neighbor_transpose(idx[:, :1].contiguous(), n0, build=True)
            if tr0 is None:
                raise NotImplementedError(_NO_TABLE.format("adaptive_weight"))
            gcen = new(n0, M)
            _lib.check(L.cbl_grouping_backward_csr_rows(_i(n0), _i(M), _i(M), _i(0), _lib.ptr(gc), _lib.ptr(tr0[0]), _lib.ptr(tr0[1]), _lib.ptr(tr0[2]),
                                                        _lib.ptr(gcen), st), "cbl_grouping_backward_csr_rows")
        return None, None, None, gf, gcen, gn, gwp, gb, ghw, ghb, None, None, None, None


_AW_MLP_M = (16, 144)


def _aw_mlp_limits(fc_num, M, K=None):
    if fc_num > 3:
        raise NotImplementedError("adaptive_weight.fc_num {}: fc_num 1, 2 and 3 are implemented".format(fc_num))
    if not _AW_MLP_M[0] <= M <= _AW_MLP_M[1]:
        raise NotImplementedError("adaptive_weight.fc_num {}: only fc_num 1 is implemented for {} weight groups (the per-pair MLP kernels take {} to {})".format(
            fc_num, M, *_AW_MLP_M))
    if K is not None and (K > 128 or (K > 48 and M > 64)):
        raise NotImplementedError("adaptive_weight.fc_num {}: {} neighbours with {} weight groups (at most 48, or 128 up to 64 groups)".format(fc_num, K, M))


def adaptive_weight(query_points, support_points, neighbors_indices, features, radius, fc_weight, fc_bias, reduction="mean", *,
                    local_input_feature="dp", shared_channels=1, weight_softmax=False, fc_hidden=(), activation_fn="relu"):
    S = _aw_options(local_input_feature, shared_channels, weight_softmax, reduction, features.shape[1])
    C = features.shape[1]
    M = C // S
    if tuple(fc_weight.shape) != (_aw_d_in(local_input_feature, C), M):
        raise ValueError("fc_weight: shape {}, local_input_feature {} of {} features with shared_channels {} has ({}, {})".format(
            tuple(fc_weight.shape), local_input_feature, C, shared_channels, _aw_d_in(local_input_feature, C), M))
    _chk(query_points, torch.float32, "query_points"); _chk(support_points, torch.float32, "support_points")
    _chk(neighbors_indices, torch.int32, "neighbors_indices"); _chk(features, torch.float32, "features")
    _chk(fc_weight, torch.float32, "fc_weight"); _chk(fc_bias, torch.float32, "fc_bias")
    softmax, red = _AW_SOFTMAX[weight_softmax], _AW_REDUCTIONS[reduction]
    fc_hidden = tuple(fc_hidden)
    if fc_hidden:
        _aw_mlp_limits(1 + len(fc_hidden), M, neighbors_indices.shape[1])
        for l, (w, b) in enumerate(fc_hidden, 1):
            _chk(w, torch.float32, "fc_hidden[{}] weight".format(l - 1)); _chk(b, torch.float32, "fc_hidden[{}] bias".format(l - 1))
            if tuple(w.shape) != (M, M) or tuple(b.shape) != (M,):
                raise ValueError("fc_hidden[{}]: shapes {} and {}, a layer of {} weight groups has ({}, {}) and ({},)".format(
                    l - 1, tuple(w.shape), tuple(b.shape), M, M, M, M))
    if not fc_hidden and local_input_feature == "dp" and S == 1 and softmax == 0 and red != 2:
        return _AdaptiveWeight.apply(query_points, support_points, neighbors_indices, features, fc_weight, fc_bias, float(radius), red)
    if C % 4 != 0 or C > 1152:
        raise NotImplementedError("adaptive_weight: {} features (a multiple of 4 up to 1152)".format(C))
    if neighbors_indices.shape[1] > 128:
        raise NotImplementedError("adaptive_weight: {} neighbours (at most 128)".format(neighbors_indices.shape[1]))
    from . import dense
    blocks, o = {}, 0
    for name in local_input_feature.split("_"):
        rows = 3 if name == "dp" else C
        blocks[name] = fc_weight[o:o + rows]
        o += rows
    w_pos = blocks["dp"].contiguous() if "dp" in blocks else None
    center_term = neighbor_term = None
    if "fi" in blocks or "df" in blocks:
        w_c = blocks["fi"] - blocks["df"] if "fi" in blocks else -blocks["df"]
        center_term = dense.linear(features, w_c.t()).contiguous()
    if "df" in blocks or "fj" in blocks:
        w_n = blocks["df"] if "df" in blocks else blocks["fj"]
        neighbor_term = dense.linear(features, w_n.t()).contiguous()
    if fc_hidden:
        return _AdaptiveWeightMLP.apply(query_points, support_points, neighbors_indices, features, center_term, neighbor_term, w_pos, fc_bias,
                                        torch.stack([w for w, _ in fc_hidden]), torch.stack([b for _, b in fc_hidden]), float(radius), softmax, red,
                                        _PW_ACTIVATIONS.get(activation_fn, 0))
    return _AdaptiveWeightGeneral.apply(query_points, support_points, neighbors_indices, features, center_term, neighbor_term, w_pos, fc_bias, float(radius),
                                        softmax, red)


def _fan_in_init_(weights):
    std = (1.3 / weights.shape[0]) ** 0.5
    with torch.no_grad():
        return torch.nn.init.trunc_normal_(weights, 0.0, std, -2 * std, 2 * std)


class AdaptiveWeight(torch.nn.Module):

    def __init__(self, in_fdim, local_input_feature="dp", shared_channels=1, fc_num=1, weight_softmax=False, reduction="mean", activation_fn="relu"):
        super().__init__()
        if fc_num < 1:
            raise ValueError("adaptive_weight.fc_num {}: at least 1".format(fc_num))
        S = _aw_options(local_input_feature, shared_channels, weight_softmax, reduction, in_fdim)
        d_in, M = _aw_d_in(local_input_feature, in_fdim), in_fdim // S
        if fc_num != 1:
            _aw_mlp_limits(fc_num, M)
        self.local_input_feature, self.shared_channels, self.fc_num = local_input_feature, shared_channels, fc_num
        self.weight_softmax, self.reduction, self.activation_fn = weight_softmax, reduction, activation_fn
        self.weights = torch.nn.Parameter(torch.empty(d_in, M))
        _fan_in_init_(self.weights)
        self.biases = torch.nn.Parameter(torch.zeros(M))
        for l in range(1, fc_num):
            w = torch.nn.Parameter(torch.empty(M, M))
            _fan_in_init_(w)
            setattr(self, "weights_{}".format(l), w)
            setattr(self, "biases_{}".format(l), torch.nn.Parameter(torch.zeros(M)))

# ... 478 lines not shown
```

include/cbl_amd.h:

```cpp
#ifndef CBL_AMD_H
#define CBL_AMD_H

#include <stddef.h>
#include <stdint.h>

#ifdef __cplusplus
extern "C" {
#endif

#define CBL_OK               0
#define CBL_ERR_BAD_ARG     (-1)
#define CBL_ERR_WORKSPACE   (-2)
#define CBL_ERR_UNSUPPORTED (-3)

#define CBL_KNN_MAX_NSAMPLE 1024
#define CBL_CONTRAST_PAIRS_MAX_D 4096

const char* cbl_version(void);
int         cbl_device_arch_ok(void);


int cbl_knnquery(int b, int n, int m, int nsample,
                 const float* xyz, const float* new_xyz,
                 const int* offset, const int* new_offset,
                 int* idx, float* dist2,
                 void* workspace, size_t workspace_bytes, void* stream);
size_t cbl_knnquery_workspace_bytes(int b, int n, int m, int nsample);

int cbl_knnquery_set(int b, int n, int m, int nsample,
                     const float* xyz, const float* new_xyz,
                     const int* offset, const int* new_offset,
                     int* idx, float* dist2,
                     void* workspace, size_t workspace_bytes, void* stream);
int cbl_knnquery_anytie(int b, int n, int m, int nsample,
                        const float* xyz, const float* new_xyz,
                        const int* offset, const int* new_offset,
                        int* idx, float* dist2,
                        void* workspace, size_t workspace_bytes, void* stream);

int cbl_knnquery_ordered(int b, int n, int m, int nsample,
                         const float* xyz, const float* new_xyz,
                         const int* offset, const int* new_offset,
                         int* idx, float* dist2, int tie_policy, int* cell_order,
                         void* workspace, size_t workspace_bytes, void* stream);

int cbl_knn_grid_block_candidates(int b, int n, int nsample, const int* offset, int* count, void* workspace, size_t workspace_bytes, void* stream);

size_t cbl_knnquery_prefix_workspace_bytes(int m);
int cbl_knnquery_prefix(int b, int n, int m, int nsample_wide, int nsample,
                        const float* xyz, const float* new_xyz, const int* offset, const int* new_offset,
                        const int* idx_wide, const float* dist2_wide, int* idx, float* dist2, int tie_policy,
                        void* workspace, size_t workspace_bytes, void* stream);

int cbl_knnquery_nested(int b, int n, int m, int nsample_wide, int tie_policy_wide, int nsample, int tie_policy,
                        const float* xyz, const float* new_xyz, const int* offset, const int* new_offset,
                        int* idx_wide, float* dist2_wide, int* idx, float* dist2, int* cell_order, void* event_after_wide,
                        void* workspace, size_t workspace_bytes, void* stream);

int cbl_knnquery_exact(int b, int n, int m, int nsample,
                       const float* xyz, const float* new_xyz,
                       const int* offset, const int* new_offset,
                       int* idx, float* dist2, void* stream);

int cbl_furthestsampling(int b, int n_max, const float* xyz, const int* offset, const int* new_offset,
                         float* tmp, int* idx, void* stream);
size_t cbl_furthestsampling_workspace_bytes(int b, int n, int n_max);
int cbl_furthestsampling_ws(int b, int n, int n_max, const float* xyz, const int* offset, const int* new_offset,
                            float* tmp, int* idx, void* workspace, size_t workspace_bytes, void* stream);
int cbl_furthestsampling_chain(int b, int n, int n_max, const float* xyz, const int* offset, const int* new_offset, float* tmp, int* idx,
                               const int* cert_in, int* cert_out, void* workspace, size_t workspace_bytes, void* stream);

int cbl_grouping_forward(int m, int nsample, int c, const float* input, const int* idx, float* output, void* stream);
int cbl_grouping_forward_ordered(int m, int nsample, int c, const float* input, const int* idx, const int* order, float* output, void* stream);
int cbl_grouping_backward(int m, int nsample, int c, const float* grad_output, const int* idx, float* grad_input, void* stream);

size_t cbl_neighbor_transpose_workspace_bytes(int m, int n, int nsample);
int cbl_neighbor_transpose(int m, int n, int nsample, const int* idx, const int* order_src, const int* order_dst, int* inv_start, int* inv_src,
                           void* workspace, size_t workspace_bytes, void* stream);
size_t cbl_neighbor_transpose_pair_workspace_bytes(int m, int n, int nsample_a, int nsample_b);
int cbl_neighbor_transpose_pair(int m, int n, int nsample_a, const int* idx_a, int nsample_b, const int* idx_b, const int* order_src, const int* order_dst,
                                int* inv_start_a, int* inv_src_a, int* inv_start_b, int* inv_src_b, void* workspace, size_t workspace_bytes, void* stream);
int cbl_grouping_backward_csr(int n, int c, const float* grad_output, const int* order_dst, const int* inv_start, const int* inv_src,
                              float* grad_input, void* stream);
int cbl_grouping_backward_csr_rows(int n, int c, int row_stride, int col_offset, const float* grad_output, const int* order_dst,
                                   const int* inv_start, const int* inv_src, float* grad_input, void* stream);
int cbl_weighted_scatter_csr(int n, int nsample, int c, int w_c, const float* rows, const float* weight, const int* order_dst, const int* inv_start,
                             const int* inv_src, float* grad_input, void* stream);
int cbl_subtraction_backward_csr(int m, int n2, int nsample, int c, const float* grad_output, const int* order_dst, const int* inv_start,
                                 const int* inv_src, float* grad_input1, float* grad_input2, void* stream);

int cbl_interpolation_forward(int n, int c, int k, const float* input, const int* idx, const float* weight, float* output, void* stream);
int cbl_interpolation_backward(int n, int c, int k, const float* grad_output, const int* idx, const float* weight, float* grad_input, void* stream);

int cbl_subtraction_forward(int n, int nsample, int c, const float* input1, const float* input2, const int* idx, float* output, void* stream);
int cbl_subtraction_forward_ordered(int n, int nsample, int c, const float* input1, const float* input2, const int* idx, const int* order,
                                    float* output, void* stream);
int cbl_subtraction_backward(int n, int nsample, int c, const int* idx, const float* grad_output, float* grad_input1, float* grad_input2, void* stream);

int cbl_aggregation_forward(int n, int nsample, int c, int w_c, const float* input, const float* position, const float* weight, const int* idx, float* output, void* stream);
int cbl_aggregation_forward_ordered(int n, int nsample, int c, int w_c, const float* input, const float* position, const float* weight, const int* idx,
                                    const int* order, float* output, void* stream);
int cbl_aggregation_backward(int n, int nsample, int c, int w_c, const float* input, const float* position, const float* weight, const int* idx, const float* grad_output, float* grad_input, float* grad_position, float* grad_weight, void* stream);


int cbl_queryandgroup(int m, int nsample, int c, int use_xyz, const float* xyz, const float* new_xyz, const float* feat, const int* idx, float* out, void* stream);
int cbl_queryandgroup_ordered(int m, int nsample, int c, int use_xyz, const float* xyz, const float* new_xyz, const float* feat, const int* idx,
                              const int* order, float* out, void* stream);

int cbl_interpolation_weights(int n, int k, const float* dist2, float* weight, float* dist, void* stream);



int cbl_subscene_label(int m, int kr, int num_classes, const long long* target, const int* neighbor_idx, float* out, void* stream);

int cbl_label_argmax(int m, int num_classes, const float* labels, int* amax, void* stream);

int cbl_point_contrast_forward(int m, int nsample, int d, const float* features, const int* amax, const int* neighbor_idx,
                               float temperature, float weight, float* per_point, int* point_mask, float* stats, float* loss, void* stream);
int cbl_point_contrast_backward(int m, int nsample, int d, const float* features, const int* amax, const int* neighbor_idx,
                                float temperature, float weight, const float* stats, const float* grad_loss, float* grad_features, void* stream);

int cbl_point_contrast_forward_grad(int m, int nsample, int d, const float* features, const int* amax, const int* neighbor_idx,
                                    float temperature, float weight, float* per_point, int* point_mask, float* stats, float* loss,
                                    float* grad_unit, void* stream);
int cbl_point_contrast_forward_l64(int m, int nsample, int d, const float* features, const long long* labels, const int* neighbor_idx,
                                   float temperature, float weight, float* per_point, int* point_mask, float* stats, float* loss, void* stream);
int cbl_point_contrast_forward_grad_l64(int m, int nsample, int d, const float* features, const long long* labels, const int* neighbor_idx,
                                        float temperature, float weight, float* per_point, int* point_mask, float* stats, float* loss,
                                        float* grad_unit, void* stream);
int cbl_tf_contrast_forward_grad(int m, int n_valid, int nsample, int d, const float* features, const int* labels, const int* neighbors,
                                 float temperature, float weight, float* per_point, int* point_mask, float* stats, float* loss,
                                 float* grad_unit, void* stream);
int cbl_tf_contrast_forward_kl(int m, int n_valid, int nsample, int d, const float* features, const float* soft_labels, int num_classes,
                               float kl_threshold, const int* neighbors, float temperature, float weight, float* per_point, int* point_mask,
                               float* stats, float* loss, void* stream);
int cbl_tf_contrast_forward_grad_kl(int m, int n_valid, int nsample, int d, const float* features, const float* soft_labels, int num_classes,
                                    float kl_threshold, const int* neighbors, float temperature, float weight, float* per_point, int* point_mask,
                                    float* stats, float* loss, float* grad_unit, void* stream);
int cbl_contrast_grad_scale(long long total, const float* grad_unit, const float* stats, const float* grad_loss, float weight,
                            float* grad_features, void* stream);

int cbl_contrast_pairs_forward(int m, int n_valid, int flags, int nsample, int d, const float* features, const void* labels, int num_classes,
                               float kl_threshold, const int* neighbor_idx, const int* order, float temperature, float weight,
                               float* per_point, int* point_mask, float* stats, float* loss, float* coef, float* grad_own, void* stream);
#define CBL_ROLE_LABEL 0
#define CBL_ROLE_POS 1
#define CBL_ROLE_NEG 2
#define CBL_ROLE_NEG_REJECT 3
int cbl_contrast_pairs_forward_samples(int m, int n_valid, int flags, int nsample, int d, const float* features, const void* labels, int num_classes,
                                       float kl_threshold, const int* sample_idx, const unsigned char* roles, const unsigned char* sample_valid,
                                       const int* order, float temperature, float weight, float* per_point, int* point_mask, float* stats,
                                       float* loss, float* coef, float* grad_own, void* stream);
int cbl_contrast_pairs_backward(int m, int nsample, int d, const float* features, const float* coef, const float* grad_own, const int* order,
                                const int* inv_start, const int* inv_src, const float* stats, const float* grad_loss, float weight,
                                float* grad_features, void* stream);

int cbl_contrast_pairs_backward_atomic(int m, int n_valid, int nsample, int d, const float* features, const float* coef, const float* grad_own,
                                       const int* neighbor_idx, const float* stats, const float* grad_loss, float weight,
                                       float* grad_features, void* stream);

int cbl_tf_contrast_forward(int m, int n_valid, int nsample, int d, const float* features, const int* labels, const int* neighbors,
                            float temperature, float weight, float* per_point, int* point_mask, float* stats, float* loss, void* stream);
int cbl_tf_contrast_backward(int m, int n_valid, int nsample, int d, const float* features, const int* labels, const int* neighbors,
                             float temperature, float weight, const float* stats, const float* grad_loss, float* grad_features, void* stream);
int cbl_tf_scene_label(int m, int n_valid, int k, int num_classes, const long long* point_labels, const int* scene_neighbor, int by_valid, float* out, void* stream);

int cbl_boundary_mask(int n, int k, const long long* labels, const int* neighbor_idx, unsigned char* bound, unsigned char* plain, int* cnt, void* stream);

int cbl_cumulate_probs(int n, int num_classes, int m, const long long* inds, const float* pred, float smooth, int mode, float* probs,
                       int* scratch_n, void* stream);

int cbl_boundary_iou(int n, int k, int num_classes, long long ignore_label, const long long* pred, const long long* labels,
                     const int* neighbor_idx, unsigned long long* hist, void* stream);


int cbl_kpconv_forward(int n, int n0, int K, int C, int KP, const float* query_points, const float* support_points, const int* neighbors_indices,
                       const float* features, const float* kernel_points, const float* kernel_weights, float extent, int influence, int closest,
                       float* out, void* stream);
int cbl_kpconv_forward_ordered(int n, int n0, int K, int C, int KP, const float* query_points, const float* support_points, const int* neighbors_indices,
                               const float* features, const float* kernel_points, const float* kernel_weights, float extent, int influence, int closest,
                               const int* order, float* out, void* stream);
int cbl_kpconv_backward(int n, int n0, int K, int C, int KP, const float* query_points, const float* support_points, const int* neighbors_indices,
                        const float* features, const float* kernel_points, const float* kernel_weights, float extent, int influence, int closest,
                        const float* grad_out, float* grad_features, float* grad_kernel_weights, void* stream);

size_t cbl_kpconv_backward_csr_workspace_bytes(int n0, int C, int KP);
int cbl_kpconv_backward_csr(int n, int n0, int K, int C, int KP, const float* query_points, const float* support_points, const float* features,
                            const float* kernel_points, const float* kernel_weights, float extent, int influence, int closest,
                            const float* grad_out, const int* order_dst, const int* inv_start, const int* inv_src,
                            float* grad_features, float* grad_kernel_weights, void* workspace, size_t workspace_bytes, void* stream);

int cbl_index_max(long long total, const int* idx, int* out_max, void* stream);
int cbl_adaptive_weight_forward(int n, int n0, int K, int C, const float* query_points, const float* support_points, const int* neighbors_indices,
                                const float* features, float radius, const float* fc_weight, const float* fc_bias, const int* padding_num,
                                int reduction_mean, float* out, void* stream);
int cbl_adaptive_weight_forward_ordered(int n, int n0, int K, int C, const float* query_points, const float* support_points, const int* neighbors_indices,
                                        const float* features, float radius, const float* fc_weight, const float* fc_bias, const int* padding_num,
                                        int reduction_mean, const int* order, float* out, void* stream);
int cbl_adaptive_weight_backward(int n, int n0, int K, int C, const float* query_points, const float* support_points, const int* neighbors_indices,
                                 const float* features, float radius, const float* fc_weight, const float* fc_bias, const int* padding_num,
                                 int reduction_mean, const float* grad_out, float* grad_features, float* grad_fc_weight, float* grad_fc_bias, void* stream);

size_t cbl_adaptive_weight_backward_csr_workspace_bytes(int n, int n0, int C);
int cbl_adaptive_weight_backward_csr(int n, int n0, int K, int C, const float* query_points, const float* support_points, const int* neighbors_indices,
                                     const float* features, float radius, const float* fc_weight, const float* fc_bias, const int* padding_num,
                                     int reduction_mean, const float* grad_out, const int* order_dst, const int* inv_start, const int* inv_src,
                                     float* grad_features, float* grad_fc_weight, float* grad_fc_bias, void* workspace, size_t workspace_bytes, void* stream);

size_t cbl_adaptive_weight_general_workspace_bytes(int n, int n0, int K, int C, int M);
int cbl_adaptive_weight_general_forward(int n, int n0, int K, int C, int M, const float* query_points, const float* support_points,
                                        const int* neighbors_indices, const float* features, const float* center_term, const float* neighbor_term,
                                        const float* w_pos, const float* bias, float radius, int softmax, int reduction, const int* padding_num,
                                        float* out, void* workspace, size_t workspace_bytes, void* stream);
int cbl_adaptive_weight_general_backward_csr(int n, int n0, int K, int C, int M, const float* query_points, const float* support_points,
                                             const int* neighbors_indices, const float* features, const float* center_term, const float* neighbor_term,
                                             const float* w_pos, const float* bias, float radius, int softmax, int reduction, const int* padding_num,
                                             const float* out, const float* grad_out, const int* order_dst, const int* inv_start, const int* inv_src,
                                             float* grad_features_value, float* grad_center, float* grad_neighbor, float* grad_w_pos, float* grad_bias,
                                             void* workspace, size_t workspace_bytes, void* stream);

size_t cbl_adaptive_weight_mlp_workspace_bytes(int n, int n0, int K, int C, int M, int layers);
int cbl_adaptive_weight_mlp_forward(int n, int n0, int K, int C, int M, const float* query_points, const float* support_points,
                                    const int* neighbors_indices, const float* features, const float* center_term, const float* neighbor_term,
                                    const float* w_pos, const float* bias, int layers, const float* hidden_w, const float* hidden_b, int activation,
                                    float radius, int softmax, int reduction, const int* padding_num, float* out, void* workspace,
                                    size_t workspace_bytes, void* stream);
int cbl_adaptive_weight_mlp_backward_csr(int n, int n0, int K, int C, int M, const float* query_points, const float* support_points,
                                         const int* neighbors_indices, const float* features, const float* center_term, const float* neighbor_term,
                                         const float* w_pos, const float* bias, int layers, const float* hidden_w, const float* hidden_b, int activation,
                                         float radius, int softmax, int reduction, const int* padding_num, const float* out, const float* grad_out,
                                         const int* order_dst, const int* inv_start, const int* inv_src, float* grad_features_value, float* grad_center,
                                         float* grad_neighbor, float* grad_w_pos, float* grad_bias, float* grad_hidden_w, float* grad_hidden_b,
                                         void* workspace, size_t workspace_bytes, void* stream);

int cbl_pospool_forward(int n, int n0, int K, int C, const float* query_points, const float* support_points, const int* neighbors_indices,
                        const float* features, float radius, int position_embedding, int reduction, const int* padding_num,
                        float* out, void* stream);
int cbl_pospool_backward(int n, int n0, int K, int C, const float* query_points, const float* support_points, const int* neighbors_indices,
                         const float* features, float radius, int position_embedding, int reduction, const int* padding_num,
                         const float* grad_out, float* grad_features, void* stream);
size_t cbl_pospool_backward_csr_workspace_bytes(int n);
int cbl_pospool_backward_csr(int n, int n0, int K, int C, const float* query_points, const float* support_points, const int* neighbors_indices,
                             float radius, int position_embedding, int reduction, const int* padding_num, const float* grad_out,
                             const int* order_dst, const int* inv_start, const int* inv_src, float* grad_features,
                             void* workspace, size_t workspace_bytes, void* stream);

size_t cbl_pointwise_mlp_workspace_bytes(int n, int n0, int K, int C_out);
int cbl_pointwise_mlp_forward(int n, int n0, int K, int C_out, const float* query_points, const float* support_points, const int* neighbors_indices,
                              const float* center_term, const float* neighbor_term, const float* w_pos, float radius,
                              int bn_mode, const float* gamma, const float* beta, float eps, float momentum, float* moving_mean, float* moving_var,
                              int activation, int reduction, const int* padding_num, float* save_mean, float* save_invstd, float* out,
                              void* workspace, size_t workspace_bytes, void* stream);
int cbl_pointwise_mlp_backward_csr(int n, int n0, int K, int C_out, const float* query_points, const float* support_points, const int* neighbors_indices,
                                   const float* center_term, const float* neighbor_term, const float* w_pos, float radius,
                                   int bn_mode, const float* gamma, const float* beta, const float* save_mean, const float* save_invstd,
                                   int activation, int reduction, const int* padding_num, const float* out, const float* grad_out,
                                   const int* order_dst, const int* inv_start, const int* inv_src,
                                   float* grad_center, float* grad_neighbor, float* grad_w_pos, float* grad_gamma, float* grad_beta,
                                   void* workspace, size_t workspace_bytes, void* stream);

size_t cbl_pointwise_mlp_layers_workspace_bytes(int n, int n0, int K, int H, int C_out, int layers);
int cbl_pointwise_mlp_layers_forward(int n, int n0, int K, int H, int C_out, const float* query_points, const float* support_points,
                                     const int* neighbors_indices, const float* center_term, const float* neighbor_term, const float* w_pos, float radius,
                                     int layers, const float* hidden_w, int bn_mode, const float* gamma, const float* beta, float eps, float momentum,
                                     float* moving_mean, float* moving_var, int activation, int reduction, const int* padding_num, float* save_mean,
                                     float* save_invstd, float* out, void* workspace, size_t workspace_bytes, void* stream);
int cbl_pointwise_mlp_layers_backward_csr(int n, int n0, int K, int H, int C_out, const float* query_points, const float* support_points,
                                          const int* neighbors_indices, const float* center_term, const float* neighbor_term, const float* w_pos,
                                          float radius, int layers, const float* hidden_w, int bn_mode, const float* gamma, const float* beta,
                                          const float* save_mean, const float* save_invstd, int activation, int reduction, const int* padding_num,
                                          const float* out, const float* grad_out, const int* order_dst, const int* inv_start, const int* inv_src,
                                          float* grad_center, float* grad_neighbor, float* grad_w_pos, float* grad_hidden_w, float* grad_gamma,
                                          float* grad_beta, void* workspace, size_t workspace_bytes, void* stream);

size_t cbl_attn_workspace_bytes(int C, int G);
int cbl_attn_w2_forward(int n, int K, int C, int G, const float* x_q, const float* x_k, const int* idx, const float* p1,
                        const float* W3C, const float* b3C, const float* bn_weight, const float* bn_bias, float eps, float momentum,
                        float* running_mean, float* running_var, long long* num_batches_tracked, int training,
                        const float* Wa, const float* ba, float* save_mean, float* save_invstd, float* w2,
                        void* workspace, size_t workspace_bytes, void* stream);
int cbl_attn_w2_backward(int n, int K, int C, int G, const float* x_q, const float* x_k, const int* idx, const float* p1,
                         const float* W3C, const float* b3C, const float* bn_weight, const float* bn_bias,
                         const float* save_mean, const float* save_invstd, const float* Wa, const float* grad_w2,
                         float* grad_xq, float* grad_xk, float* grad_p1, float* grad_W3C, float* grad_b3C,
                         float* grad_bn_weight, float* grad_bn_bias, float* grad_Wa, float* grad_ba,
                         void* workspace, size_t workspace_bytes, void* stream);
int cbl_attn_agg_forward(int n, int K, int C, int G, const float* x_v, const int* idx, const float* p1, const float* W3C, const float* b3C,
                         const float* a, float* out, void* stream);
int cbl_attn_agg_backward(int n, int K, int C, int G, const float* x_v, const int* idx, const float* p1, const float* W3C, const float* b3C,
                          const float* a, const float* grad_out, float* grad_xv, float* grad_p1, float* grad_W3C, float* grad_b3C, float* grad_a,
                          void* workspace, size_t workspace_bytes, void* stream);
int cbl_attn_agg_softmax_forward(int n, int K, int C, int G, const float* x_v, const int* idx, const float* p1, const float* W3C, const float* b3C,
                                 const float* logits, float* a, float* out, void* stream);
int cbl_attn_agg_softmax_backward(int n, int K, int C, int G, const float* x_v, const int* idx, const float* p1, const float* W3C, const float* b3C,
                                  const float* a, const float* grad_out, float* grad_xv, float* grad_p1, float* grad_W3C, float* grad_b3C,
                                  float* grad_logits, void* workspace, size_t workspace_bytes, void* stream);

int cbl_attn_w2_backward_csr(int n, int K, int C, int G, const float* x_q, const float* x_k, const int* idx, const float* p1,
                             const float* W3C, const float* b3C, const float* bn_weight, const float* bn_bias,
                             const float* save_mean, const float* save_invstd, const float* Wa, const float* grad_w2,
                             const int* order, const int* inv_start, const int* inv_src,
                             float* grad_xq, float* grad_xk, float* grad_p1, float* grad_W3C, float* grad_b3C,
                             float* grad_bn_weight, float* grad_bn_bias, float* grad_Wa, float* grad_ba,
                             void* workspace, size_t workspace_bytes, void* stream);
int cbl_attn_agg_backward_csr(int n, int K, int C, int G, const float* x_v, const int* idx, const float* p1, const float* W3C, const float* b3C,
                              const float* a, const float* grad_out, const int* order, const int* inv_start, const int* inv_src,
                              float* grad_xv, float* grad_p1, float* grad_W3C, float* grad_b3C, float* grad_a,
                              void* workspace, size_t workspace_bytes, int softmax, void* stream);
int cbl_attn_w2_backward_wide_csr(int n, int K, int C, int G, const float* x_q, const float* x_k, const int* idx, const float* p1,
                                  const float* W3C, const float* b3C, const float* bn_weight, const float* bn_bias,
                                  const float* save_mean, const float* save_invstd, const float* Wa, const float* grad_w2,
                                  const int* order, const int* inv_start, const int* inv_src,
                                  float* grad_xq, float* grad_xk, float* grad_p1, float* grad_W3C, float* grad_b3C,
                                  float* grad_bn_weight, float* grad_bn_bias, float* grad_Wa, float* grad_ba,
                                  void* workspace, size_t workspace_bytes, void* stream);
int cbl_attn_agg_backward_wide_csr(int n, int K, int C, int G, const float* x_v, const int* idx, const float* p1, const float* W3C, const float* b3C,
                                   const float* a, const float* grad_out, const int* order, const int* inv_start, const int* inv_src,
                                   float* grad_xv, float* grad_p1, float* grad_W3C, float* grad_b3C, float* grad_a,
                                   void* workspace, size_t workspace_bytes, int softmax, void* stream);

size_t cbl_pt_layer_workspace_bytes(int n, int K, int C);
int cbl_pt_layer_consts_floats(void);
size_t cbl_pt_layer_wide_workspace_bytes(int n, int K, int C);
int cbl_pt_layer_wide_consts_floats(void);
int cbl_pt_layer_wide_forward(int n, int K, int C, const float* xyz, const float* x_q, const float* x_k, const float* x_v, const int* idx,
                              const float* Wp, const float* bp, const float* gamma_p, const float* beta_p, const float* W3C, const float* b3C,
                              const float* gamma_c, const float* beta_c, const float* Wa, const float* ba, const float* gamma_g, const float* beta_g,
                              const float* Wb, const float* bb, const float* eps3, const float* momentum3, float* const* running_mean3,
                              float* const* running_var3, long long* const* num_batches3, float* p_r, float* p0, float* p1, float* w2, float* a, float* out,
                              float* consts, float* bnc_stats, void* workspace, size_t workspace_bytes, void* stream);
int cbl_pt_layer_wide_backward(int n, int K, int C, const float* x_q, const float* x_k, const float* x_v, const int* idx, const float* gamma_p,
                               const float* W3C, const float* b3C, const float* gamma_c, const float* beta_c, const float* Wa, const float* gamma_g,
                               const float* Wb, const float* p_r, const float* p0, const float* p1, const float* w2, const float* a, const float* consts,
                               const float* bnc_stats, const float* grad_out, float* g_xq, float* g_xk, float* g_xv, float* g_Wp, float* g_bp,
                               float* g_gamma_p, float* g_beta_p, float* g_W3C, float* g_b3C, float* g_gamma_c, float* g_beta_c, float* g_Wa, float* g_ba,
                               float* g_gamma_g, float* g_beta_g, float* g_Wb, float* g_bb, void* workspace, size_t workspace_bytes, void* stream);
int cbl_pt_layer_wide_backward_csr(int n, int K, int C, const float* x_q, const float* x_k, const float* x_v, const int* idx,
                                   const int* order, const int* inv_start, const int* inv_src, const float* gamma_p,
                                   const float* W3C, const float* b3C, const float* gamma_c, const float* beta_c, const float* Wa, const float* gamma_g,
                                   const float* Wb, const float* p_r, const float* p0, const float* p1, const float* w2, const float* a, const float* consts,
                                   const float* bnc_stats, const float* grad_out, float* g_xq, float* g_xk, float* g_xv, float* g_Wp, float* g_bp,
                                   float* g_gamma_p, float* g_beta_p, float* g_W3C, float* g_b3C, float* g_gamma_c, float* g_beta_c, float* g_Wa, float* g_ba,
                                   float* g_gamma_g, float* g_beta_g, float* g_Wb, float* g_bb, void* workspace, size_t workspace_bytes, void* stream);

int cbl_pt_layer_selftest_chain(const float* A, const float* B, const float* C, float* d_mfma, float* d_fma, void* stream);
int cbl_pt_layer_forward(int n, int K, int C, const float* xyz, const float* x_q, const float* x_k, const float* x_v, const int* idx, const int* order,
                         const float* Wp, const float* bp, const float* gamma_p, const float* beta_p, const float* W3C, const float* b3C,
                         const float* gamma_c, const float* beta_c, const float* Wa, const float* ba, const float* gamma_g, const float* beta_g,
                         const float* Wb, const float* bb, const float* eps3, const float* momentum3, float* const* running_mean3,
                         float* const* running_var3, long long* const* num_batches3, float* p_r, float* p0, float* p1, float* w2, float* a, float* out,
                         float* consts, void* workspace, size_t workspace_bytes, void* stream);
int cbl_pt_layer_forward_eval(int n, int K, int C, const float* xyz, const float* x_q, const float* x_k, const float* x_v, const int* idx, const int* order,
                              const float* Wp, const float* bp, const float* gamma_p, const float* beta_p, const float* W3C, const float* b3C,
                              const float* gamma_c, const float* beta_c, const float* Wa, const float* ba, const float* gamma_g, const float* beta_g,
                              const float* Wb, const float* bb, const float* eps3, const float* const* running_mean3, const float* const* running_var3,
                              float* p_r, float* p0, float* p1, float* w2, float* a, float* out, float* consts, void* workspace, size_t workspace_bytes,
                              void* stream);
int cbl_pt_layer_backward(int n, int K, int C, const float* x_q, const float* x_k, const float* x_v, const int* idx, const int* order,
                          const int* inv_start, const int* inv_src, const float* gamma_p, const float* W3C, const float* b3C, const float* gamma_c,
                          const float* Wa, const float* gamma_g, const float* Wb, const float* p_r, const float* p0, const float* p1, const float* w2,
                          const float* a, const float* consts, const float* grad_out, float* g_xq, float* g_xk, float* g_xv, float* g_Wp, float* g_bp,
                          float* g_gamma_p, float* g_beta_p, float* g_W3C, float* g_b3C, float* g_gamma_c, float* g_beta_c, float* g_Wa, float* g_ba,
                          float* g_gamma_g, float* g_beta_g, float* g_Wb, float* g_bb, void* workspace, size_t workspace_bytes, void* stream);

size_t cbl_skinny_linear_workspace_bytes(int cin, int cout);
int cbl_skinny_linear_forward(long long rows, int cin, int cout, const float* x, const float* weight, const float* bias, float* y, void* stream);
int cbl_skinny_linear_backward_input(long long rows, int cin, int cout, const float* grad_y, const float* weight, float* grad_x, void* stream);
int cbl_skinny_linear_backward_weight(long long rows, int cin, int cout, const float* x, const float* grad_y, float* grad_weight, float* grad_bias,
                                      void* workspace, size_t workspace_bytes, void* stream);

size_t cbl_triple_linear_workspace_bytes(int C);
int cbl_triple_linear_forward(long long rows, int C, const float* x, const float* const* weight3, const float* const* bias3, float* const* y3, void* stream);
int cbl_triple_linear_backward(long long rows, int C, const float* x, const float* const* weight3, const float* const* grad_y3, float* grad_x,
                               float* const* grad_weight3, float* const* grad_bias3, void* workspace, size_t workspace_bytes, void* stream);

size_t cbl_bn_rows_workspace_bytes(long long rows, int C);
int cbl_bn_rows_forward(long long rows, int C, const float* x, const float* weight, const float* bias, float eps, float momentum,
                        float* running_mean, float* running_var, long long* num_batches_tracked, int relu, float* save_mean, float* save_invstd,
                        float* y, void* workspace, size_t workspace_bytes, void* stream);
int cbl_bn_rows_backward(long long rows, int C, const float* x, const float* grad_y, const float* weight, const float* bias,
                         const float* save_mean, const float* save_invstd, int relu, float* grad_x, float* grad_weight, float* grad_bias,
                         void* workspace, size_t workspace_bytes, void* stream);
int cbl_bn_rows_forward_residual(long long rows, int C, const float* x, const float* residual, const float* weight, const float* bias, float eps, float momentum,
                                 float* running_mean, float* running_var, long long* num_batches_tracked, int relu, float* save_mean, float* save_invstd,
                                 float* y, void* workspace, size_t workspace_bytes, void* stream);
int cbl_bn_rows_backward_residual(long long rows, int C, const float* x, const float* residual, const float* grad_y, const float* weight, const float* bias,
                                  const float* save_mean, const float* save_invstd, int relu, float* grad_x, float* grad_residual, float* grad_weight,
                                  float* grad_bias, void* workspace, size_t workspace_bytes, void* stream);

size_t cbl_cross_entropy_workspace_bytes(long long n);
int cbl_cross_entropy_forward(long long n, int k, const float* logits, const long long* target, long long ignore_index, float* loss, float* stats,
                              void* workspace, size_t workspace_bytes, void* stream);
int cbl_cross_entropy_backward(long long n, int k, const float* logits, const long long* target, long long ignore_index, const float* stats,
                               const float* grad_loss, float* grad_logits, void* stream);

int cbl_ind_max_pool(int n1, int n2, int k, int d, const float* x, const int* inds, unsigned* scratch_d, float* out, void* stream);
int cbl_ind_closest_pool(int n1, int n2, int k, int d, const float* x, const int* inds, float* out, void* stream);
size_t cbl_ind_max_pool_backward_workspace_bytes(int n1, int n2, int k, int d);
int cbl_ind_max_pool_backward_csr(int n1, int n2, int k, int d, const float* x, const int* inds, const unsigned* keymin_d,
                                  const float* out, const float* grad_out, const int* order, const int* inv_start, const int* inv_src,
                                  float* grad_x, void* ws, size_t ws_bytes, void* stream);


size_t cbl_grid_subsampling_workspace_bytes(int b, int n);
int cbl_grid_subsampling(int b, int n, const float* points, const int* offset, float dl,
                         int fdim, const float* features, int ldim, const int* labels,
                         float* out_points, float* out_features, int* out_labels, int* out_lengths, int* out_total,
                         void* workspace, size_t workspace_bytes, void* stream);

size_t cbl_radius_neighbors_workspace_bytes(int b, int ns);
int cbl_radius_neighbors(int b, int nq, int ns, const float* queries, const float* supports, const int* q_offset, const int* s_offset,
                         float radius, int limit, int* out, int* counts, int* max_count, void* workspace, size_t workspace_bytes, void* stream);
int cbl_radius_neighbors_reuse(int b, int nq, int ns, const float* queries, const float* supports, const int* q_offset, const int* s_offset,
                               float radius, int limit, int* out, int* counts, int* max_count, void* workspace, size_t workspace_bytes,
                               int grid_is_built, void* stream);

size_t cbl_pyramid_layer_workspace_bytes(int b, int n);
int cbl_pyramid_layer(int b, int n, const float* points, const int* lengths, float radius, float sample_dl, int limit,
                      void* grid_ws, size_t grid_ws_bytes, int grid_is_built,
                      int* neighbors, float* pool_points, int* pool_lengths, int* pools, int* upsamples,
                      void* next_grid_ws, size_t next_grid_ws_bytes, int* max_counts, int* host_pool_points,
                      void* workspace, size_t workspace_bytes, void* stream);

int cbl_pyramid(int b, int n, const float* points, const int* lengths, float radius0, float dl0, int num_layers, const int* limits,
                void* const* grid_ws, size_t grid_ws_bytes, int* const* neighbors, float* const* pool_points, int* const* pool_lengths,
                int* const* pools, int* const* upsamples, int* max_counts, int* host_sizes, void* workspace, size_t workspace_bytes, void* stream);

typedef struct CblConvnetLayer {
    int n, K, C, Kp, d;
    float radius;
    const float* points;
    const int* neighbors;
    const float* features;
    const float* fc_weight;
    const float* fc_bias;
    const float* grad_out;
    const float* latent;
    const int* pools;
    float* aw_out;
    float* grad_features;
    float* grad_fc_weight;
    float* grad_fc_bias;
    float* cbl_loss;
    int* cbl_mask;
    float* grad_latent;
    int* labels;
} CblConvnetLayer;
size_t cbl_convnet_step_workspace_bytes(int nlayers, const CblConvnetLayer* layers, int num_classes);
int cbl_convnet_step(int nlayers, const CblConvnetLayer* layers, const long long* point_labels, int num_classes, float temperature, float weight,
                     void* workspace, size_t workspace_bytes, void* stream);

int cbl_knn_indices_to_local(int B, int M, int K, int N, const int* idx, long long* out, void* stream);


size_t cbl_voxelize_workspace_bytes(int n);
int cbl_voxelize(int n, int is_f64, const void* coord, double voxel_size, unsigned long long* keys_sorted, int* idx_sort,
                 int* start, int* count, int* num_voxels, void* workspace, size_t workspace_bytes, void* stream);

int cbl_crop_order(int n, int is_f64, const void* coord, int center, int* order, void* workspace, size_t workspace_bytes, void* stream);

#ifdef __cplusplus
}
#endif
#endif
```

Before: 146.7 million.

## Fuse query-and-group and KPConv forward into one role-split kernel launch

After: 152.5 million (median of 6 runs). 1.04x the previous value.

```diff
diff --git a/contrastboundary_amd/build.py b/contrastboundary_amd/build.py
--- a/contrastboundary_amd/build.py
+++ b/contrastboundary_amd/build.py
@@ -26,7 +26,7 @@
     return hs
 
 
-EXTRA_FLAGS = {"local_aggregation.hip": ["-mllvm", "-amdgpu-mfma-vgpr-form"]}
+EXTRA_FLAGS = {"local_aggregation.hip": ["-mllvm", "-amdgpu-mfma-vgpr-form"], "block_roles.hip": ["-mllvm", "-amdgpu-mfma-vgpr-form"]}
 
 def _compile(src, obj, verbose):
     tmp = obj + ".tmp.%d" % os.getpid()
diff --git a/contrastboundary_amd/csrc/block_roles.hip b/contrastboundary_amd/csrc/block_roles.hip
--- /dev/null
+++ b/contrastboundary_amd/csrc/block_roles.hip
@@ -0,0 +1,101 @@
+#include "cbl_common.h"
+#include <atomic>
+
+namespace {
+
+using f32x4 = __attribute__((ext_vector_type(4))) float;
+
+#include "query_group_pipe.h"
+#include "kpconv_fwd_c64.h"
+
+struct CblRoles { unsigned num, den; };
+struct CblRoleSlot { bool a; unsigned id, count; };
+
+__host__ __device__ inline unsigned cbl_roles_count_a(unsigned per, CblRoles r) { const unsigned rem = per % r.den; return (per / r.den) * r.num + (rem < r.num ? rem : r.num); }
+
+__device__ __forceinline__ CblRoleSlot cbl_role_slot(unsigned b, unsigned grid, CblRoles r)
+{
+    const unsigned per = grid >> 3, i = b >> 3, x = b & 7u, q = i / r.den, rem = i - q * r.den, na = cbl_roles_count_a(per, r);
+    CblRoleSlot s;
+    s.a = rem < r.num;
+    s.id = 8u * (s.a ? q * r.num + rem : q * (r.den - r.num) + (rem - r.num)) + x;
+    s.count = 8u * (s.a ? na : per - na);
+    return s;
+}
+
+template <int C4T, int PR, bool CLOSEST, bool LINEAR>
+__global__ __launch_bounds__(256) void block_fwd_roles_kernel(CblRoles roles, unsigned npieces, const float* __restrict__ xyz, const float* __restrict__ new_xyz,
+                                                              const float4* __restrict__ feat, const int* __restrict__ gidx, const int* __restrict__ gorder,
+                                                              float* __restrict__ grouped, int n, int n0, int K, int C, int KP, const float* __restrict__ q,
+                                                              const float* __restrict__ s, const int* __restrict__ idx, const float* __restrict__ f,
+                                                              const float* __restrict__ kpts, const float* __restrict__ kw, float extent,
+                                                              const int* __restrict__ order, float* __restrict__ out)
+{
+    const CblRoleSlot slot = cbl_role_slot(blockIdx.x, gridDim.x, roles);
+    if (slot.a) query_group_lds_pipe_body<C4T, PR>(slot.id, slot.count, npieces, xyz, new_xyz, feat, gidx, gorder, grouped);
+    else        kpconv_fwd_c64_body<CLOSEST, LINEAR, true>(slot.id, slot.count, n, n0, K, C, KP, q, s, idx, f, kpts, kw, extent, order, out);
+}
+
+struct RolesConfig { std::atomic<int> num, den, max_blocks; };
+RolesConfig roles_config[1] = {{{0}, {0}, {0}}};
+constexpr CblRoles ROLES_DEFAULT[1] = {{1u, 3u}};
+
+CblRoles roles_of(int pass)
+{
+    const int num = roles_config[pass].num.load(), den = roles_config[pass].den.load();
+    if (num > 0 && den > num) return CblRoles{(unsigned)num, (unsigned)den};
+    return ROLES_DEFAULT[pass];
+}
+
+unsigned roles_grid(int pass, const void* kernel, unsigned nwg_a, unsigned nwg_b, CblRoles r)
+{
+    const unsigned period = 8u * r.den;
+    unsigned g = cbl_resident_blocks(kernel, 256, 0);
+    const unsigned long long want = ((unsigned long long)nwg_a + nwg_b + period - 1) / period * period;
+    if (want < g) g = (unsigned)want;
+    const int cap = roles_config[pass].max_blocks.load();
+    if (cap > 0 && (unsigned)cap < g) g = (unsigned)cap;
+    g &= ~7u;
+    return g < period ? period : g;
+}
+
+}
+
+CBL_EXPORT int cbl_block_roles_config(int pass, int share_num, int share_den, int max_blocks)
+{
+    if (pass != 0 || share_num < 0 || share_den < 0 || max_blocks < 0 || (share_den > 0 && !(share_num > 0 && share_num < share_den))) return CBL_ERR_BAD_ARG;
+    if (share_den > 64) return CBL_ERR_BAD_ARG;
+    roles_config[pass].num.store(share_num); roles_config[pass].den.store(share_den); roles_config[pass].max_blocks.store(max_blocks);
+    return CBL_OK;
+}
+
+CBL_EXPORT int cbl_group_kpconv_forward_ordered(int m, int nsample, int c, int use_xyz, const float* xyz, const float* new_xyz, const float* feat, const int* idx,
+                                                const int* group_order, float* grouped,
+                                                int n, int n0, int K, int C, int KP, const float* query_points, const float* support_points,
+                                                const int* neighbors_indices, const float* features, const float* kernel_points, const float* kernel_weights,
+                                                float extent, int influence, int closest, const int* order, float* out, void* stream)
+{
+    const bool gather_ok = m > 0 && nsample == 16 && c == 64 && use_xyz && xyz && new_xyz && feat && idx && group_order && grouped &&
+                           cbl_host_aligned16(feat) && cbl_host_aligned16(grouped) && (long long)m * nsample < 0xffffffffLL;
+    const bool kpconv_ok = n > 0 && n0 > 0 && K == 16 && C == 64 && KP > 0 && KP <= 16 && extent > 0.f && influence == 1 && closest == 0 &&
+                           query_points && support_points && neighbors_indices && features && kernel_points && kernel_weights && out &&
+                           cbl_host_aligned16(features) && cbl_host_aligned16(out) && cbl_host_aligned16(kernel_weights) &&
+                           (unsigned long long)n0 * C * 4ull < (1ull << 32);
+    if (gather_ok && kpconv_ok) {
+        const CblRoles r = roles_of(0);
+        const void* kernel = reinterpret_cast<const void*>(&block_fwd_roles_kernel<16, 16, false, true>);
+        const unsigned g = roles_grid(0, kernel, ((unsigned)m + 3u) / 4u, ((unsigned)n + 3u) / 4u, r);
+        hipLaunchKernelGGL((block_fwd_roles_kernel<16, 16, false, true>), dim3(g), dim3(256), 0, cbl_stream(stream), r, (unsigned)m, xyz, new_xyz,
+                           reinterpret_cast<const float4*>(feat), idx, group_order, grouped, n, n0, K, C, KP, query_points, support_points, neighbors_indices,
+                           features, kernel_points, kernel_weights, extent, order, out);
+        return cbl_status();
+    }
+#ifdef CBL_HOST_WAVE_EMULATION
+    return CBL_ERR_UNSUPPORTED;
+#else
+    const int rc = cbl_queryandgroup_ordered(m, nsample, c, use_xyz, xyz, new_xyz, feat, idx, group_order, grouped, stream);
+    if (rc != CBL_OK) return rc;
+    return cbl_kpconv_forward_ordered(n, n0, K, C, KP, query_points, support_points, neighbors_indices, features, kernel_points, kernel_weights, extent, influence,
+                                      closest, order, out, stream);
+#endif
+}
diff --git a/contrastboundary_amd/csrc/kpconv_fwd_c64.h b/contrastboundary_amd/csrc/kpconv_fwd_c64.h
--- /dev/null
+++ b/contrastboundary_amd/csrc/kpconv_fwd_c64.h
@@ -0,0 +1,157 @@
+#pragma once
+
+__device__ __forceinline__ float rows_sum4(float x)
+{
+    const unsigned u = __float_as_uint(x);
+    const auto a = __builtin_amdgcn_permlane16_swap(u, u, false, false);
+    const float y = __uint_as_float(a[0]) + __uint_as_float(a[1]);
+    const unsigned w = __float_as_uint(y);
+    const auto b = __builtin_amdgcn_permlane32_swap(w, w, false, false);
+    return __uint_as_float(b[0]) + __uint_as_float(b[1]);
+}
+
+template <bool CLOSEST, bool LINEAR, bool ONE>
+__device__ __forceinline__ void kpconv_fwd_c64_body(unsigned bid, unsigned nblk, int n, int n0, int K, int C, int KP, const float* __restrict__ q,
+                                                    const float* __restrict__ s, const int* __restrict__ idx, const float* __restrict__ f,
+                                                    const float* __restrict__ kpts, const float* __restrict__ kw, float extent,
+                                                    const int* __restrict__ order, float* __restrict__ out)
+{
+    __shared__ float4 kw_s[16 * 16];
+    {
+        const int row = threadIdx.x >> 4, col = threadIdx.x & 15;
+        kw_s[threadIdx.x] = (row < KP && 4 * col < C) ? *reinterpret_cast<const float4*>(kw + (size_t)row * C + 4 * col) : make_float4(0.f, 0.f, 0.f, 0.f);
+    }
+    __syncthreads();
+    const int lane = threadIdx.x & 63;
+    const int kp_id = lane & 15, kq = lane >> 4;
+    const unsigned wv = __builtin_amdgcn_readfirstlane(threadIdx.x >> 6), nwg = ((unsigned)n + 3u) >> 2;
+    const bool kp_ok = kp_id < KP;
+    const float kx = kp_ok ? kpts[3 * kp_id] : 0.f, ky = kp_ok ? kpts[3 * kp_id + 1] : 0.f, kz = kp_ok ? kpts[3 * kp_id + 2] : 0.f;
+    const float inv_extent = 1.0f / extent;
+    const float m2kx = -2.f * kx, m2ky = -2.f * ky, m2kz = -2.f * kz, k2 = (kx * kx + ky * ky) + kz * kz;
+    const int cb = 4 * kp_id;
+    const bool ch_ok = cb < C;
+    const char* fbytes = reinterpret_cast<const char*>(f);
+    const unsigned row_bytes = 4u * (unsigned)C, col_bytes = 4u * (unsigned)(ch_ok ? cb : 0);
+    const unsigned vend = 8 * cbl_xcd_per(nwg), vstep = nblk;
+    auto point_at = [&](unsigned v) -> int {
+        if (v >= vend) return -1;
+        const unsigned t = (order ? cbl_xcd_slot(v, nwg) : v) * 4 + wv;
+        return t < (unsigned)n ? (order ? order[t] : (int)t) : -1;
+    };
+    struct Xyz { float x, y, z, qx, qy, qz; };
+    struct Rows { float4 v[4]; bool real[4]; };
+    auto load_ids = [&](int pt) -> int { return (pt >= 0 && lane < K) ? idx[(size_t)pt * K + lane] : n0; };
+    auto load_xyz = [&](int pt, int id) -> Xyz {
+        Xyz g;
+        const bool real = id >= 0 && id < n0;
+        const float3 sp = *reinterpret_cast<const float3*>(s + 3 * (size_t)(real ? id : 0));
+        g.x = real ? sp.x : 1e6f; g.y = real ? sp.y : 1e6f; g.z = real ? sp.z : 1e6f;
+        const float3 qp = *reinterpret_cast<const float3*>(q + 3 * (size_t)(pt >= 0 ? pt : 0));
+        g.qx = qp.x; g.qy = qp.y; g.qz = qp.z;
+        return g;
+    };
+    auto load_rows = [&](int ids, int kc) -> Rows {
+        Rows r;
+#pragma unroll
+        for (int gi = 0; gi < 4; gi++) {
+            const int id = __shfl(ids, (kc + 4 * gi + kq) & 63);
+            r.real[gi] = id >= 0 && id < n0;
+            r.v[gi] = *reinterpret_cast<const float4*>(fbytes + ((unsigned)(r.real[gi] ? id : 0) * row_bytes + col_bytes));
+        }
+        return r;
+    };
+    const f32x4 zero = {0.f, 0.f, 0.f, 0.f};
+    auto chunk = [&](const Rows& rows, int kc, float mrx, float mry, float mrz, float mr2, f32x4 (&acc)[4], bool first) {
+        float a[4];
+#pragma unroll
+        for (int gi = 0; gi < 4; gi++) {
+            const int src = (kc + 4 * gi + kq) & 63;
+            const float rx = __shfl(mrx, src), ry = __shfl(mry, src), rz = __shfl(mrz, src);
+            float sq;
+            if (CLOSEST) {
+                const float dx = rx - kx, dy = ry - ky, dz = rz - kz;
+                sq = (dx * dx + dy * dy) + dz * dz;
+            } else {
+                const float r2 = __shfl(mr2, src);
+                sq = fmaxf(__builtin_fmaf(m2kx, rx, __builtin_fmaf(m2ky, ry, __builtin_fmaf(m2kz, rz, r2 + k2))), 0.f);
+            }
+            float w = LINEAR ? fmaxf(1.0f - __builtin_amdgcn_sqrtf(sq) * inv_extent, 0.0f) : 1.0f;
+            if (CLOSEST) {
+                float bs = kp_ok ? sq : INFINITY; int bi = kp_id;
+#pragma unroll
+                for (int sft = 8; sft >= 1; sft >>= 1) {
+                    const float os = __shfl_xor(bs, sft, 16); const int oi = __shfl_xor(bi, sft, 16);
+                    if (os < bs || (os == bs && oi < bi)) { bs = os; bi = oi; }
+                }
+                if (bi != kp_id) w = 0.f;
+            }
+            a[gi] = (kp_ok && rows.real[gi]) ? w : 0.f;
+        }
+#pragma unroll
+        for (int gi = 0; gi < 4; gi++) {
+            const bool z = first && gi == 0;
+            const bool rl = rows.real[gi];
+            acc[0] = __builtin_amdgcn_mfma_f32_16x16x4f32(a[gi], rl ? rows.v[gi].x : 0.f, z ? zero : acc[0], 0, 0, 0);
+            acc[1] = __builtin_amdgcn_mfma_f32_16x16x4f32(a[gi], rl ? rows.v[gi].y : 0.f, z ? zero : acc[1], 0, 0, 0);
+            acc[2] = __builtin_amdgcn_mfma_f32_16x16x4f32(a[gi], rl ? rows.v[gi].z : 0.f, z ? zero : acc[2], 0, 0, 0);
+            acc[3] = __builtin_amdgcn_mfma_f32_16x16x4f32(a[gi], rl ? rows.v[gi].w : 0.f, z ? zero : acc[3], 0, 0, 0);
+        }
+    };
+    int p0 = point_at(bid), p1 = point_at(bid + vstep), p2 = point_at(bid + 2 * vstep);
+    int id0 = load_ids(p0), id1 = load_ids(p1);
+    Xyz g0 = load_xyz(p0, id0);
+    Rows r0 = load_rows(id0, 0);
+    for (unsigned v = bid; v < vend; v += vstep) {
+        const int p3 = point_at(v + 3 * vstep);
+        const int p = p0;
+        const int id2 = load_ids(p2); const Xyz g1 = load_xyz(p1, id1); const Rows r1 = load_rows(id1, 0);
+        __builtin_amdgcn_sched_barrier(0);
+        if (p >= 0) {
+            const float mrx = g0.x - g0.qx, mry = g0.y - g0.qy, mrz = g0.z - g0.qz;
+            const float mr2 = (mrx * mrx + mry * mry) + mrz * mrz;
+            f32x4 acc[4];
+#pragma unroll
+            for (int t = 0; t < 4; t++) acc[t] = zero;
+            chunk(r0, 0, mrx, mry, mrz, mr2, acc, true);
+            if (!ONE) {
+                for (int k0 = 0; k0 < K; k0 += 64) {
+                    int ids = id0; float cx = mrx, cy = mry, cz = mrz, c2 = mr2;
+                    if (k0 > 0) {
+                        ids = (k0 + lane < K) ? idx[(size_t)p * K + k0 + lane] : n0;
+                        const bool real = ids >= 0 && ids < n0;
+                        const float3 sp = *reinterpret_cast<const float3*>(s + 3 * (size_t)(real ? ids : 0));
+                        cx = (real ? sp.x : 1e6f) - g0.qx; cy = (real ? sp.y : 1e6f) - g0.qy; cz = (real ? sp.z : 1e6f) - g0.qz;
+                        c2 = (cx * cx + cy * cy) + cz * cz;
+                    }
+                    for (int kc = (k0 == 0 ? 16 : 0); kc < min(64, K - k0); kc += 16) {
+                        const Rows rr = load_rows(ids, kc);
+                        chunk(rr, kc, cx, cy, cz, c2, acc, false);
+                    }
+                }
+            }
+            float res[4];
+#pragma unroll
+            for (int t = 0; t < 4; t++) res[t] = 0.f;
+#pragma unroll
+            for (int r = 0; r < 4; r++) {
+                const float4 k4 = kw_s[(kq * 4 + r) * 16 + kp_id];
+                res[0] = __builtin_fmaf(k4.x, acc[0][r], res[0]); res[1] = __builtin_fmaf(k4.y, acc[1][r], res[1]);
+                res[2] = __builtin_fmaf(k4.z, acc[2][r], res[2]); res[3] = __builtin_fmaf(k4.w, acc[3][r], res[3]);
+            }
+#pragma unroll
+            for (int t = 0; t < 4; t++) res[t] = rows_sum4(res[t]);
+            if (lane < 16 && ch_ok) *reinterpret_cast<float4*>(out + (size_t)p * C + cb) = make_float4(res[0], res[1], res[2], res[3]);
+        }
+        p0 = p1; p1 = p2; p2 = p3; id0 = id1; id1 = id2; g0 = g1; r0 = r1;
+    }
+}
+
+template <bool CLOSEST, bool LINEAR, bool ONE>
+__global__ __launch_bounds__(256) void kpconv_fwd_c64_kernel(int n, int n0, int K, int C, int KP, const float* __restrict__ q,
+                                                             const float* __restrict__ s, const int* __restrict__ idx, const float* __restrict__ f,
+                                                             const float* __restrict__ kpts, const float* __restrict__ kw, float extent,
+                                                             const int* __restrict__ order, float* __restrict__ out)
+{
+    kpconv_fwd_c64_body<CLOSEST, LINEAR, ONE>(blockIdx.x, gridDim.x, n, n0, K, C, KP, q, s, idx, f, kpts, kw, extent, order, out);
+}
diff --git a/contrastboundary_amd/csrc/local_aggregation.hip b/contrastboundary_amd/csrc/local_aggregation.hip
--- a/contrastboundary_amd/csrc/local_aggregation.hip
+++ b/contrastboundary_amd/csrc/local_aggregation.hip
@@ -126,152 +126,7 @@
     }
 }
 
-__device__ __forceinline__ float rows_sum4(float x)
-{
-    const unsigned u = __float_as_uint(x);
-    const auto a = __builtin_amdgcn_permlane16_swap(u, u, false, false);
-    const float y = __uint_as_float(a[0]) + __uint_as_float(a[1]);
-    const unsigned w = __float_as_uint(y);
-    const auto b = __builtin_amdgcn_permlane32_swap(w, w, false, false);
-    return __uint_as_float(b[0]) + __uint_as_float(b[1]);
-}
-
-template <bool CLOSEST, bool LINEAR, bool ONE>
-__global__ __launch_bounds__(256) void kpconv_fwd_c64_kernel(int n, int n0, int K, int C, int KP, const float* __restrict__ q,
-                                                             const float* __restrict__ s, const int* __restrict__ idx, const float* __restrict__ f,
-                                                             const float* __restrict__ kpts, const float* __restrict__ kw, float extent,
-                                                             const int* __restrict__ order, float* __restrict__ out)
-{
-    __shared__ float4 kw_s[16 * 16];
-    {
-        const int row = threadIdx.x >> 4, col = threadIdx.x & 15;
-        kw_s[threadIdx.x] = (row < KP && 4 * col < C) ? *reinterpret_cast<const float4*>(kw + (size_t)row * C + 4 * col) : make_float4(0.f, 0.f, 0.f, 0.f);
-    }
-    __syncthreads();
-    const int lane = threadIdx.x & 63;
-    const int kp_id = lane & 15, kq = lane >> 4;
-    const unsigned wv = __builtin_amdgcn_readfirstlane(threadIdx.x >> 6), nwg = ((unsigned)n + 3u) >> 2;
-    const bool kp_ok = kp_id < KP;
-    const float kx = kp_ok ? kpts[3 * kp_id] : 0.f, ky = kp_ok ? kpts[3 * kp_id + 1] : 0.f, kz = kp_ok ? kpts[3 * kp_id + 2] : 0.f;
-    const float inv_extent = 1.0f / extent;
-    const float m2kx = -2.f * kx, m2ky = -2.f * ky, m2kz = -2.f * kz, k2 = (kx * kx + ky * ky) + kz * kz;
-    const int cb = 4 * kp_id;
-    const bool ch_ok = cb < C;
-    const char* fbytes = reinterpret_cast<const char*>(f);
-    const unsigned row_bytes = 4u * (unsigned)C, col_bytes = 4u * (unsigned)(ch_ok ? cb : 0);
-    const unsigned vend = 8 * cbl_xcd_per(nwg), vstep = gridDim.x;
-    auto point_at = [&](unsigned v) -> int {
-        if (v >= vend) return -1;
-        const unsigned t = (order ? cbl_xcd_slot(v, nwg) : v) * 4 + wv;
-        return t < (unsigned)n ? (order ? order[t] : (int)t) : -1;
-    };
-    struct Xyz { float x, y, z, qx, qy, qz; };
-    struct Rows { float4 v[4]; bool real[4]; };
-    auto load_ids = [&](int pt) -> int { return (pt >= 0 && lane < K) ? idx[(size_t)pt * K + lane] : n0; };
-    auto load_xyz = [&](int pt, int id) -> Xyz {
-        Xyz g;
-        const bool real = id >= 0 && id < n0;
-        const float3 sp = *reinterpret_cast<const float3*>(s + 3 * (size_t)(real ? id : 0));
-        g.x = real ? sp.x : 1e6f; g.y = real ? sp.y : 1e6f; g.z = real ? sp.z : 1e6f;
-        const float3 qp = *reinterpret_cast<const float3*>(q + 3 * (size_t)(pt >= 0 ? pt : 0));
-        g.qx = qp.x; g.qy = qp.y; g.qz = qp.z;
-        return g;
-    };
-    auto load_rows = [&](int ids, int kc) -> Rows {
-        Rows r;
-#pragma unroll
-        for (int gi = 0; gi < 4; gi++) {
-            const int id = __shfl(ids, (kc + 4 * gi + kq) & 63);
-            r.real[gi] = id >= 0 && id < n0;
-            r.v[gi] = *reinterpret_cast<const float4*>(fbytes + ((unsigned)(r.real[gi] ? id : 0) * row_bytes + col_bytes));
-        }
-        return r;
-    };
-    const f32x4 zero = {0.f, 0.f, 0.f, 0.f};
-    auto chunk = [&](const Rows& rows, int kc, float mrx, float mry, float mrz, float mr2, f32x4 (&acc)[4], bool first) {
-        float a[4];
-#pragma unroll
-        for (int gi = 0; gi < 4; gi++) {
-            const int src = (kc + 4 * gi + kq) & 63;
-            const float rx = __shfl(mrx, src), ry = __shfl(mry, src), rz = __shfl(mrz, src);
-            float sq;
-            if (CLOSEST) {
-                const float dx = rx - kx, dy = ry - ky, dz = rz - kz;
-                sq = (dx * dx + dy * dy) + dz * dz;
-            } else {
-                const float r2 = __shfl(mr2, src);
-                sq = fmaxf(__builtin_fmaf(m2kx, rx, __builtin_fmaf(m2ky, ry, __builtin_fmaf(m2kz, rz, r2 + k2))), 0.f);
-            }
-            float w = LINEAR ? fmaxf(1.0f - __builtin_amdgcn_sqrtf(sq) * inv_extent, 0.0f) : 1.0f;
-            if (CLOSEST) {
-                float bs = kp_ok ? sq : INFINITY; int bi = kp_id;
-#pragma unroll
-                for (int sft = 8; sft >= 1; sft >>= 1) {
-                    const float os = __shfl_xor(bs, sft, 16); const int oi = __shfl_xor(bi, sft, 16);
-                    if (os < bs || (os == bs && oi < bi)) { bs = os; bi = oi; }
-                }
-                if (bi != kp_id) w = 0.f;
-            }
-            a[gi] = (kp_ok && rows.real[gi]) ? w : 0.f;
-        }
-#pragma unroll
-        for (int gi = 0; gi < 4; gi++) {
-            const bool z = first && gi == 0;
-            const bool rl = rows.real[gi];
-            acc[0] = __builtin_amdgcn_mfma_f32_16x16x4f32(a[gi], rl ? rows.v[gi].x : 0.f, z ? zero : acc[0], 0, 0, 0);
-            acc[1] = __builtin_amdgcn_mfma_f32_16x16x4f32(a[gi], rl ? rows.v[gi].y : 0.f, z ? zero : acc[1], 0, 0, 0);
-            acc[2] = __builtin_amdgcn_mfma_f32_16x16x4f32(a[gi], rl ? rows.v[gi].z : 0.f, z ? zero : acc[2], 0, 0, 0);
-            acc[3] = __builtin_amdgcn_mfma_f32_16x16x4f32(a[gi], rl ? rows.v[gi].w : 0.f, z ? zero : acc[3], 0, 0, 0);
-        }
-    };
-    int p0 = point_at(blockIdx.x), p1 = point_at(blockIdx.x + vstep), p2 = point_at(blockIdx.x + 2 * vstep);
-    int id0 = load_ids(p0), id1 = load_ids(p1);
-    Xyz g0 = load_xyz(p0, id0);
-    Rows r0 = load_rows(id0, 0);
-    for (unsigned v = blockIdx.x; v < vend; v += vstep) {
-        const int p3 = point_at(v + 3 * vstep);
-        const int p = p0;
-        const int id2 = load_ids(p2); const Xyz g1 = load_xyz(p1, id1); const Rows r1 = load_rows(id1, 0);
-        __builtin_amdgcn_sched_barrier(0);
-        if (p >= 0) {
-            const float mrx = g0.x - g0.qx, mry = g0.y - g0.qy, mrz = g0.z - g0.qz;
-            const float mr2 = (mrx * mrx + mry * mry) + mrz * mrz;
-            f32x4 acc[4];
-#pragma unroll
-            for (int t = 0; t < 4; t++) acc[t] = zero;
-            chunk(r0, 0, mrx, mry, mrz, mr2, acc, true);
-            if (!ONE) {
-                for (int k0 = 0; k0 < K; k0 += 64) {
-                    int ids = id0; float cx = mrx, cy = mry, cz = mrz, c2 = mr2;
-                    if (k0 > 0) {
-                        ids = (k0 + lane < K) ? idx[(size_t)p * K + k0 + lane] : n0;
-                        const bool real = ids >= 0 && ids < n0;
-                        const float3 sp = *reinterpret_cast<const float3*>(s + 3 * (size_t)(real ? ids : 0));
-                        cx = (real ? sp.x : 1e6f) - g0.qx; cy = (real ? sp.y : 1e6f) - g0.qy; cz = (real ? sp.z : 1e6f) - g0.qz;
-                        c2 = (cx * cx + cy * cy) + cz * cz;
-                    }
-                    for (int kc = (k0 == 0 ? 16 : 0); kc < min(64, K - k0); kc += 16) {
-                        const Rows rr = load_rows(ids, kc);
-                        chunk(rr, kc, cx, cy, cz, c2, acc, false);
-                    }
-                }
-            }
-            float res[4];
-#pragma unroll
-            for (int t = 0; t < 4; t++) res[t] = 0.f;
-#pragma unroll
-            for (int r = 0; r < 4; r++) {
-                const float4 k4 = kw_s[(kq * 4 + r) * 16 + kp_id];
-                res[0] = __builtin_fmaf(k4.x, acc[0][r], res[0]); res[1] = __builtin_fmaf(k4.y, acc[1][r], res[1]);
-                res[2] = __builtin_fmaf(k4.z, acc[2][r], res[2]); res[3] = __builtin_fmaf(k4.w, acc[3][r], res[3]);
-            }
-#pragma unroll
-            for (int t = 0; t < 4; t++) res[t] = rows_sum4(res[t]);
-            if (lane < 16 && ch_ok) *reinterpret_cast<float4*>(out + (size_t)p * C + cb) = make_float4(res[0], res[1], res[2], res[3]);
-        }
-        p0 = p1; p1 = p2; p2 = p3; id0 = id1; id1 = id2; g0 = g1; r0 = r1;
-    }
-}
+#include "kpconv_fwd_c64.h"
 
 constexpr int KPB_MAXKP = 16, KPB_MAXK = 64;
 __global__ __launch_bounds__(256) void kpconv_bwd_kernel(int n, int n0, int K, int C, int KP, const float* __restrict__ q,
diff --git a/contrastboundary_amd/csrc/query_group_pipe.h b/contrastboundary_amd/csrc/query_group_pipe.h
--- a/contrastboundary_amd/csrc/query_group_pipe.h
+++ b/contrastboundary_amd/csrc/query_group_pipe.h
@@ -4,16 +4,16 @@
 constexpr int QGP_WAVES = 4;
 
 template <int C4T, int PR>
-__global__ __launch_bounds__(256) void query_group_lds_pipe(unsigned npieces, const float* __restrict__ xyz, const float* __restrict__ new_xyz,
-                                                            const float4* __restrict__ feat, const int* __restrict__ idx, const int* __restrict__ order,
-                                                            float* __restrict__ out)
+__device__ __forceinline__ void query_group_lds_pipe_body(unsigned bid, unsigned nblk, unsigned npieces, const float* __restrict__ xyz,
+                                                          const float* __restrict__ new_xyz, const float4* __restrict__ feat, const int* __restrict__ idx,
+                                                          const int* __restrict__ order, float* __restrict__ out)
 {
     constexpr int oc = 4 * C4T + 3, NF4 = PR * C4T, NL = (NF4 + 63) / 64, NCH = PR * oc / 4, NS = (NCH + 63) / 64, NC = (3 * PR + 63) / 64;
     static_assert((PR * oc) % 4 == 0 && NF4 % 64 == 0, "pieces are whole 16-byte chunks, feature parts whole wave loads");
     __shared__ __attribute__((aligned(16))) float qg_lds[QGP_WAVES * PR * oc];
     const int lane = threadIdx.x & 63, wv = gw_uniform((int)(threadIdx.x >> 6));
     float* piece = qg_lds + wv * PR * oc;
-    const unsigned nwg = (npieces + 3) >> 2, vend = 8 * cbl_xcd_per(nwg), vstep = gridDim.x;
+    const unsigned nwg = (npieces + 3) >> 2, vend = 8 * cbl_xcd_per(nwg), vstep = nblk;
     auto piece_of = [&](unsigned v) -> int {
         const unsigned t = (v < vend ? cbl_xcd_slot(v, nwg) : 0u) * 4 + wv;
         const bool ok = v < vend && t < npieces;
@@ -49,13 +49,13 @@
             if (e < 3 * PR) piece[row * oc + a] = cs[h] - cq[h];
         }
     };
-    int p0 = piece_of(blockIdx.x), p1 = piece_of(blockIdx.x + vstep), p2 = piece_of(blockIdx.x + 2 * vstep);
+    int p0 = piece_of(bid), p1 = piece_of(bid + vstep), p2 = piece_of(bid + 2 * vstep);
     int id1 = ids_of(p1);
     load_piece(ids_of(p0), p0);
     park();
     int pc = p0;
-    p0 = p1; { const int idn = id1; p1 = p2; id1 = ids_of(p1); p2 = piece_of(blockIdx.x + 3 * vstep); load_piece(idn, p0); }
-    for (unsigned vv = blockIdx.x; vv < vend; vv += vstep) {
+    p0 = p1; { const int idn = id1; p1 = p2; id1 = ids_of(p1); p2 = piece_of(bid + 3 * vstep); load_piece(idn, p0); }
+    for (unsigned vv = bid; vv < vend; vv += vstep) {
         gw_wave_sync();
         {
             float* o = out + (size_t)(pc < 0 ? 0 : pc) * PR * oc;
@@ -74,3 +74,11 @@
         load_piece(idn, p0);
     }
 }
+
+template <int C4T, int PR>
+__global__ __launch_bounds__(256) void query_group_lds_pipe(unsigned npieces, const float* __restrict__ xyz, const float* __restrict__ new_xyz,
+                                                            const float4* __restrict__ feat, const int* __restrict__ idx, const int* __restrict__ order,
+                                                            float* __restrict__ out)
+{
+    query_group_lds_pipe_body<C4T, PR>(blockIdx.x, gridDim.x, npieces, xyz, new_xyz, feat, idx, order, out);
+}
diff --git a/contrastboundary_amd/hotpath.py b/contrastboundary_amd/hotpath.py
--- a/contrastboundary_amd/hotpath.py
+++ b/contrastboundary_amd/hotpath.py
@@ -55,7 +55,7 @@
 SIDE_STAGES = ("cbl_knnquery_k%d" % CBL_NSAMPLE,)
 
 
-def stages(scene, k=16, backward=False, pair_tables=False):
+def stages(scene, k=16, backward=False, pair_tables=False, block_roles=None):
     n, c = scene.n, scene.c
     st = []
     leaf = (lambda t: t.detach().requires_grad_(True)) if backward else (lambda t: t)
@@ -66,14 +66,22 @@
         s["idx"], s["dist2"] = pointops.knnquery_raw(k, scene.xyz, scene.xyz, scene.offset, scene.offset)
     st.append(("knnquery_k%d" % k, knn, 12 * n + 12 * n + 8 * n * k, 8.0 * n * n))
 
+    roles = local_aggregation.block_roles(block_roles)
+    extent = 0.12
+
     def group(s):
         s["feat_leaf"], s["kw_leaf"] = leaf(scene.feat), leaf(scene.kernel_weights)
+        if roles:
+            s["feat_leaf_kpconv"] = leaf(scene.feat)
+            s["grouped"], s["kpconv"] = local_aggregation.group_kpconv(k, scene.xyz, scene.xyz, s["feat_leaf"], s["idx"], scene.xyz, s["feat_leaf_kpconv"],
+                                                                       scene.kernel_points, s["kw_leaf"], extent, roles=True)
+            return
         s["grouped"] = pointops.queryandgroup(k, scene.xyz, scene.xyz, s["feat_leaf"], s["idx"], scene.offset, scene.offset, use_xyz=True)
     st.append(("queryandgroup", group, 4 * n * k + 12 * n + 12 * n + 4 * n * c + 4 * n * k * (3 + c), 3.0 * n * k))
 
-    extent = 0.12
-
     def kpconv(s):
+        if roles:
+            return
         s["kpconv"] = local_aggregation.kpconv(scene.xyz, scene.xyz, s["idx"], s["feat_leaf"], scene.kernel_points, s["kw_leaf"], extent)
     st.append(("kpconv_fwd", kpconv, 12 * n + 12 * n + 4 * n * c + 4 * n * k + 4 * n * c, 2.0 * n * k * KP * c + 2.0 * n * KP * c))
 
@@ -104,10 +112,17 @@
     st.append(("neighbor_transpose_k%d" % k, transpose, 8 * n * k + 4 * (n + 1), 0.0))
 
     def group_bwd(s):
+        if roles:
+            up = scene.upstream(k)
+            s["grad_feat_group"], s["grad_feat_kpconv"], s["grad_kernel_weights"] = torch.autograd.grad(
+                (s["grouped"], s["kpconv"]), (s["feat_leaf"], s["feat_leaf_kpconv"], s["kw_leaf"]), (up["grad_grouped"], up["grad_kpconv"]))
+            return
         s["grad_feat_group"], = torch.autograd.grad(s["grouped"], s["feat_leaf"], scene.upstream(k)["grad_grouped"])
     st.append(("queryandgroup_bwd", group_bwd, 4 * n * k + 4 * n * k * c + 4 * n * c, 1.0 * n * k * c))
 
     def kpconv_bwd(s):
+        if roles:
+            return
         s["grad_feat_kpconv"], s["grad_kernel_weights"] = torch.autograd.grad(s["kpconv"], (s["feat_leaf"], s["kw_leaf"]), scene.upstream(k)["grad_kpconv"])
     st.append(("kpconv_bwd", kpconv_bwd, 12 * n + 12 * n + 4 * n * c + 4 * n * k + 4 * n * c + 4 * n * c + 4 * KP * c,
                2.0 * (2.0 * n * k * KP * c + 2.0 * n * KP * c)))
diff --git a/contrastboundary_amd/local_aggregation.py b/contrastboundary_amd/local_aggregation.py
--- a/contrastboundary_amd/local_aggregation.py
+++ b/contrastboundary_amd/local_aggregation.py
@@ -35,34 +35,39 @@
 
     @staticmethod
     def backward(ctx, grad_out):
-        q, s, idx, f, kp, kw = ctx.saved_tensors
-        extent, influence, closest = ctx.cfg
-        n, K = idx.shape
-        n0, C = f.shape
-        grad_out = grad_out.contiguous()
-        L = _lib.lib()
-        from . import pointops
-        tr = None
-        if C % 4 == 0:
-            tr = pointops.neighbor_transpose(idx, n0, build=pointops._build_table(n * K))
-        if tr is not None:
-            order, inv_start, inv_src = tr
-            gf = torch.empty_like(f) if ctx.needs_input_grad[3] else None
-            gkw = torch.empty_like(kw) if ctx.needs_input_grad[5] else None
-            need = L.cbl_kpconv_backward_csr_workspace_bytes(_i(n0), _i(C), _i(kp.shape[0])) if gkw is not None else 0
-            ws = torch.empty(max(need, 1), dtype=torch.uint8, device=f.device)
-            rc = L.cbl_kpconv_backward_csr(_i(n), _i(n0), _i(K), _i(C), _i(kp.shape[0]), _lib.ptr(q), _lib.ptr(s), _lib.ptr(f), _lib.ptr(kp), _lib.ptr(kw),
-                                           _f(extent), _i(influence), _i(closest), _lib.ptr(grad_out), _lib.ptr(order), _lib.ptr(inv_start), _lib.ptr(inv_src),
-                                           _lib.ptr(gf), _lib.ptr(gkw), _lib.ptr(ws), ctypes.c_size_t(ws.numel()), _lib.stream_of(f))
-            if rc != _lib.ERR_UNSUPPORTED:
-                _lib.check(rc, "cbl_kpconv_backward_csr")
-                return None, None, None, gf, None, gkw, None, None, None
-        gf = torch.zeros_like(f) if ctx.needs_input_grad[3] else None
-        gkw = torch.zeros_like(kw) if ctx.needs_input_grad[5] else None
-        _lib.check(L.cbl_kpconv_backward(_i(n), _i(n0), _i(K), _i(C), _i(kp.shape[0]), _lib.ptr(q), _lib.ptr(s), _lib.ptr(idx), _lib.ptr(f),
-                                         _lib.ptr(kp), _lib.ptr(kw), _f(extent), _i(influence), _i(closest), _lib.ptr(grad_out),
-                                         _lib.ptr(gf), _lib.ptr(gkw), _lib.stream_of(f)), "cbl_kpconv_backward")
+        gf, gkw = _kpconv_backward(ctx.saved_tensors, ctx.cfg, grad_out, ctx.needs_input_grad[3], ctx.needs_input_grad[5])
         return None, None, None, gf, None, gkw, None, None, None
+
+
+def _kpconv_backward(saved, cfg, grad_out, need_gf, need_gkw):
+    q, s, idx, f, kp, kw = saved
+    extent, influence, closest = cfg
+    n, K = idx.shape
+    n0, C = f.shape
+    grad_out = grad_out.contiguous()
+    L = _lib.lib()
+    from . import pointops
+    tr = None
+    if C % 4 == 0:
+        tr = pointops.neighbor_transpose(idx, n0, build=pointops._build_table(n * K))
+    if tr is not None:
+        order, inv_start, inv_src = tr
+        gf = torch.empty_like(f) if need_gf else None
+        gkw = torch.empty_like(kw) if need_gkw else None
+        need = L.cbl_kpconv_backward_csr_workspace_bytes(_i(n0), _i(C), _i(kp.shape[0])) if gkw is not None else 0
+        ws = torch.empty(max(need, 1), dtype=torch.uint8, device=f.device)
+        rc = L.cbl_kpconv_backward_csr(_i(n), _i(n0), _i(K), _i(C), _i(kp.shape[0]), _lib.ptr(q), _lib.ptr(s), _lib.ptr(f), _lib.ptr(kp), _lib.ptr(kw),
+                                       _f(extent), _i(influence), _i(closest), _lib.ptr(grad_out), _lib.ptr(order), _lib.ptr(inv_start), _lib.ptr(inv_src),
+                                       _lib.ptr(gf), _lib.ptr(gkw), _lib.ptr(ws), ctypes.c_size_t(ws.numel()), _lib.stream_of(f))
+        if rc != _lib.ERR_UNSUPPORTED:
+            _lib.check(rc, "cbl_kpconv_backward_csr")
+            return gf, gkw
+    gf = torch.zeros_like(f) if need_gf else None
+    gkw = torch.zeros_like(kw) if need_gkw else None
+    _lib.check(L.cbl_kpconv_backward(_i(n), _i(n0), _i(K), _i(C), _i(kp.shape[0]), _lib.ptr(q), _lib.ptr(s), _lib.ptr(idx), _lib.ptr(f),
+                                     _lib.ptr(kp), _lib.ptr(kw), _f(extent), _i(influence), _i(closest), _lib.ptr(grad_out),
+                                     _lib.ptr(gf), _lib.ptr(gkw), _lib.stream_of(f)), "cbl_kpconv_backward")
+    return gf, gkw
 
 
 def kpconv(query_points, support_points, neighbors_indices, features, kernel_points, kernel_weights, extent,
@@ -76,6 +81,76 @@
         raise ValueError("Unknown convolution mode. Should be 'closest' or 'sum'")
     return _KPConv.apply(query_points, support_points, neighbors_indices, features, kernel_points, kernel_weights, float(extent),
                          1 if KP_influence == "linear" else 0, 1 if convolution_mode == "closest" else 0)
+
+
+BLOCK_ROLES_DEFAULT = True
+
+
+def block_roles(setting=None):
+    if setting is None:
+        import os
+        env = os.environ.get("CBL_BLOCK_ROLES")
+        return BLOCK_ROLES_DEFAULT if env is None or env == "" else env != "0"
+    return bool(setting)
+
+
+class _GroupKPConv(Function):
+
+    @staticmethod
+    def forward(ctx, feat_group, feat_kpconv, kernel_weights, xyz, new_xyz, idx, support_points, kernel_points, extent, influence, closest, roles):
+        from . import pointops
+        m, nsample = idx.shape
+        c = feat_group.shape[1]
+        n0, C = feat_kpconv.shape
+        KP = kernel_points.shape[0]
+        L = _lib.lib()
+        grouped = torch.empty((m, nsample, c + 3), dtype=torch.float32, device=feat_group.device)
+        out = torch.empty((m, C), dtype=torch.float32, device=feat_kpconv.device)
+        order = pointops.spatial_order(new_xyz)
+        g_args = (_i(m), _i(nsample), _i(c), _i(1), _lib.ptr(xyz), _lib.ptr(new_xyz), _lib.ptr(feat_group), _lib.ptr(idx), _lib.ptr(order), _lib.ptr(grouped))
+        k_args = (_i(m), _i(n0), _i(nsample), _i(C), _i(KP), _lib.ptr(new_xyz), _lib.ptr(support_points), _lib.ptr(idx), _lib.ptr(feat_kpconv),
+                  _lib.ptr(kernel_points), _lib.ptr(kernel_weights), _f(extent), _i(influence), _i(closest), _lib.ptr(order), _lib.ptr(out),
+                  _lib.stream_of(feat_group))
+        if roles:
+            _lib.check(L.cbl_group_kpconv_forward_ordered(*g_args, *k_args), "cbl_group_kpconv_forward_ordered")
+        else:
+            _lib.check(L.cbl_queryandgroup_ordered(*g_args, _lib.stream_of(feat_group)), "cbl_queryandgroup")
+            _lib.check(L.cbl_kpconv_forward_ordered(*k_args), "cbl_kpconv_forward")
+        ctx.save_for_backward(new_xyz, support_points, idx, feat_kpconv, kernel_points, kernel_weights)
+        ctx.cfg = (extent, influence, closest)
+        ctx.group_dims = (feat_group.shape[0], c)
+        ctx.set_materialize_grads(False)
+        return grouped, out
+
+    @staticmethod
+    def backward(ctx, grad_grouped, grad_out):
+        from . import pointops
+        saved = ctx.saved_tensors
+        n_feat, c = ctx.group_dims
+        g_group = g_feat = g_kw = None
+        if grad_grouped is not None and ctx.needs_input_grad[0]:
+            g_group = pointops._scatter_rows(grad_grouped.contiguous(), saved[2], n_feat, 3, c)
+        if grad_out is not None and (ctx.needs_input_grad[1] or ctx.needs_input_grad[2]):
+            g_feat, g_kw = _kpconv_backward(saved, ctx.cfg, grad_out, ctx.needs_input_grad[1], ctx.needs_input_grad[2])
+        return (g_group, g_feat, g_kw) + (None,) * 9
+
+
+def group_kpconv(nsample, xyz, new_xyz, feat_group, idx, support_points, feat_kpconv, kernel_points, kernel_weights, extent,
+                 KP_influence="linear", convolution_mode="sum", roles=None):
+    if new_xyz is None:
+        new_xyz = xyz
+    for t, name in ((xyz, "xyz"), (new_xyz, "new_xyz"), (feat_group, "feat_group"), (support_points, "support_points"), (feat_kpconv, "feat_kpconv"),
+                    (kernel_points, "kernel_points"), (kernel_weights, "kernel_weights")):
+        _chk(t, torch.float32, name)
+    _chk(idx, torch.int32, "idx")
+    if idx.dim() != 2 or idx.shape[1] != nsample or idx.shape[0] != new_xyz.shape[0]:
+        raise ValueError("idx: expected (m, nsample) for the m rows of new_xyz")
+    if KP_influence not in ("linear", "constant"):
+        raise NotImplementedError("KP_influence 'gaussian': radius_gaussian is not defined in the reference")
+    if convolution_mode not in ("sum", "closest"):
+        raise ValueError("Unknown convolution mode. Should be 'closest' or 'sum'")
+    return _GroupKPConv.apply(feat_group, feat_kpconv, kernel_weights, xyz, new_xyz, idx, support_points, kernel_points, float(extent),
+                              1 if KP_influence == "linear" else 0, 1 if convolution_mode == "closest" else 0, block_roles(roles))
 
 
 class _AdaptiveWeight(Function):
diff --git a/include/cbl_amd.h b/include/cbl_amd.h
--- a/include/cbl_amd.h
+++ b/include/cbl_amd.h
@@ -180,6 +180,12 @@
 int cbl_kpconv_forward_ordered(int n, int n0, int K, int C, int KP, const float* query_points, const float* support_points, const int* neighbors_indices,
                                const float* features, const float* kernel_points, const float* kernel_weights, float extent, int influence, int closest,
                                const int* order, float* out, void* stream);
+int cbl_group_kpconv_forward_ordered(int m, int nsample, int c, int use_xyz, const float* xyz, const float* new_xyz, const float* feat, const int* idx,
+                                     const int* group_order, float* grouped,
+                                     int n, int n0, int K, int C, int KP, const float* query_points, const float* support_points,
+                                     const int* neighbors_indices, const float* features, const float* kernel_points, const float* kernel_weights,
+                                     float extent, int influence, int closest, const int* order, float* out, void* stream);
+int cbl_block_roles_config(int pass, int share_num, int share_den, int max_blocks);
 int cbl_kpconv_backward(int n, int n0, int K, int C, int KP, const float* query_points, const float* support_points, const int* neighbors_indices,
                         const float* features, const float* kernel_points, const float* kernel_weights, float extent, int influence, int closest,
                         const float* grad_out, float* grad_features, float* grad_kernel_weights, void* stream);
```
